# sarpel/wakeword_trainer_home

Measured on AMD Instinct MI355X. Metric: training samples/sec (16kHz x 1.5s clips), higher is better.
Workload: dtype bf16; 1 GPU; BASELINE config 2: cnn_small + log-mel(40) + SpecAugment, fwd/bwd + clip + AdamW, 16 kHz x 1.5 s clips resident in HBM; batch_per_gpu=512, activation_storage=bf16, arithmetic=f32, global_batch=512, n_samples=24000, parallelism=single, ranks_seen=1, hip_graph=False

## Files before the change

### wakeword_trainer_home_amd/csrc/ww_conv_fwd.hip

```cpp
#include "ww_internal.h"
#include "ww_act.h"

namespace {

typedef float floatx16 __attribute__((ext_vector_type(16)));

__device__ __forceinline__ float bnrelu(float y, float s, float t) {
    const float z = fmaf(y, s, t);
    return z < 0.f ? 0.f : z;
}

__device__ __forceinline__ void reduce_stats_slots(float s0, float s1, float q0, float q1, float *sh ,
                                                   float *__restrict__ partial_row) {
    const int tid = threadIdx.x, slot = tid >> 5, cl = tid & 31;
    __syncthreads();
    sh[slot * 128 + 2 * cl] = s0;
    sh[slot * 128 + 2 * cl + 1] = s1;
    sh[slot * 128 + 64 + 2 * cl] = q0;
    sh[slot * 128 + 64 + 2 * cl + 1] = q1;
    __syncthreads();
    if (tid < 128) {
        float t = 0.f;
#pragma unroll
        for (int s = 0; s < 8; ++s) t += sh[s * 128 + tid];
        partial_row[tid] = t;
    }
}

template <typename T>
__global__ __launch_bounds__(256) void k_stem_fwd(const float *__restrict__ x, const float *__restrict__ w, int B,
                                                  int Hin, int Win, int Ho, int Wo, T *__restrict__ y,
                                                  float *__restrict__ partials, int rev) {
    __shared__ float sh[32 * 128];
    extern __shared__ float xs[];
    const int tid = threadIdx.x, px = tid >> 3, c8 = tid & 7;
    const int ld = Win + 2;
    float wr[8][9];
#pragma unroll
    for (int j = 0; j < 8; ++j)
#pragma unroll
        for (int t = 0; t < 9; ++t) wr[j][t] = w[(8 * c8 + j) * 9 + t];
    float s[8], q[8];
#pragma unroll
    for (int j = 0; j < 8; ++j) { s[j] = 0.f; q[j] = 0.f; }
    const long npairs = (long)B * ((Ho + 1) / 2);
    float pre[4];
    auto fetch = [&](long item) {
        if (rev) item = npairs - 1 - item;
        const int fb_ = (int)(item / ((Ho + 1) / 2)), foh = 2 * (int)(item - (long)fb_ * ((Ho + 1) / 2));
        const float *xb = x + (size_t)fb_ * Hin * Win;
#pragma unroll
        for (int k = 0; k < 4; ++k) {
            const int i = tid + 256 * k;
            const int r = i / ld, c = i - r * ld;
            const int ih = 2 * foh - 1 + r, iw = c - 1;
            pre[k] = (i < 5 * ld && ih >= 0 && ih < Hin && iw >= 0 && iw < Win) ? xb[(size_t)ih * Win + iw] : 0.f;
        }
    };
    const bool ahead = 5 * ld <= 4 * 256;
    if (ahead && (long)blockIdx.x < npairs) fetch(blockIdx.x);
    for (long pr = blockIdx.x; pr < npairs; pr += gridDim.x) {
        const long prm = rev ? npairs - 1 - pr : pr;
        const int b = (int)(prm / ((Ho + 1) / 2)), oh0 = 2 * (int)(prm - (long)b * ((Ho + 1) / 2));
        __syncthreads();
        if (ahead) {
#pragma unroll
            for (int k = 0; k < 4; ++k)
                if (tid + 256 * k < 5 * ld) xs[tid + 256 * k] = pre[k];
        } else {
            const float *xb = x + (size_t)b * Hin * Win;
            for (int i = tid; i < 5 * ld; i += 256) {
                const int r = i / ld, c = i - r * ld;
                const int ih = 2 * oh0 - 1 + r, iw = c - 1;
                xs[i] = (ih >= 0 && ih < Hin && iw >= 0 && iw < Win) ? xb[(size_t)ih * Win + iw] : 0.f;
            }
        }
        __syncthreads();
        if (ahead && pr + gridDim.x < npairs) fetch(pr + gridDim.x);
        const int nrow = min(2, Ho - oh0);
        for (int it = px; it < nrow * Wo; it += 32) {
            const int rr = it >= Wo ? 1 : 0, ow = it - rr * Wo;
            float acc[8];
#pragma unroll
            for (int j = 0; j < 8; ++j) acc[j] = 0.f;
#pragma unroll
            for (int kh = 0; kh < 3; ++kh)
#pragma unroll
                for (int kw = 0; kw < 3; ++kw) {
                    const float v = xs[(2 * rr + kh) * ld + 2 * ow + kw];
#pragma unroll
                    for (int j = 0; j < 8; ++j) acc[j] = fmaf(v, wr[j][kh * 3 + kw], acc[j]);
                }
            T *dst = y + (((size_t)b * Ho + oh0 + rr) * Wo + ow) * 64 + 8 * c8;
            float4 o0 = Act<T>::round4(make_float4(acc[0], acc[1], acc[2], acc[3]));
            float4 o1 = Act<T>::round4(make_float4(acc[4], acc[5], acc[6], acc[7]));
            Act<T>::st8(dst, o0, o1);
            s[0] += o0.x; s[1] += o0.y; s[2] += o0.z; s[3] += o0.w; s[4] += o1.x; s[5] += o1.y; s[6] += o1.z; s[7] += o1.w;
            q[0] = fmaf(o0.x, o0.x, q[0]); q[1] = fmaf(o0.y, o0.y, q[1]); q[2] = fmaf(o0.z, o0.z, q[2]); q[3] = fmaf(o0.w, o0.w, q[3]);
            q[4] = fmaf(o1.x, o1.x, q[4]); q[5] = fmaf(o1.y, o1.y, q[5]); q[6] = fmaf(o1.z, o1.z, q[6]); q[7] = fmaf(o1.w, o1.w, q[7]);
        }
    }
    if (partials) {
        __syncthreads();
#pragma unroll
        for (int j = 0; j < 8; ++j) {
            sh[px * 128 + 8 * c8 + j] = s[j];
            sh[px * 128 + 64 + 8 * c8 + j] = q[j];
        }
        __syncthreads();
        if (tid < 128) {
            float t = 0.f;
#pragma unroll 8
            for (int i = 0; i < 32; ++i) t += sh[i * 128 + tid];
            partials[(size_t)blockIdx.x * 128 + tid] = t;
        }
    }
}

struct DwGeom {
    int B, H, W, ncs, nseg, hs_len;
    long items;
};

constexpr int DW_HS = 20;

template <typename T>
__device__ __forceinline__ void dw_issue_row(const T *__restrict__ img, int h, int w0, int H, int W, int cl,
                                             typename Act<T>::raw2 (&raw)[6]) {
    const int hh = min(max(h, 0), H - 1);
#pragma unroll
    for (int i = 0; i < 6; ++i) {
        const int wc = min(max(w0 - 1 + i, 0), W - 1);
        raw[i] = Act<T>::ldraw2(img + (uint32_t)((hh * W + wc) * 64 + 2 * cl));
    }
}
template <typename T>
__device__ __forceinline__ void dw_finish_row(const typename Act<T>::raw2 (&raw)[6], int h, int w0, int H, int W,
                                              float2 sc, float2 sf, float2 (&r)[6]) {
    const bool hv = (h >= 0) && (h < H);
#pragma unroll
    for (int i = 0; i < 6; ++i) {
        const int wc = w0 - 1 + i;
        const bool ok = hv && wc >= 0 && wc < W;
        const float2 v = Act<T>::cvt2(raw[i]);
        r[i].x = ok ? bnrelu(v.x, sc.x, sf.x) : 0.f;
        r[i].y = ok ? bnrelu(v.y, sc.y, sf.y) : 0.f;
    }
}

template <typename T>
__device__ __forceinline__ void dw_out_row(T *__restrict__ oimg, int h, int w0, int W, int cl,
                                           const float2 (&top)[6], const float2 (&mid)[6], const float2 (&bot)[6],
                                           const float (&wa)[9], const float (&wb)[9], float &s0, float &s1, float &q0,
                                           float &q1) {
#pragma unroll
    for (int i = 0; i < 4; ++i) {
        float a0 = 0.f, a1 = 0.f;
#pragma unroll
        for (int kw = 0; kw < 3; ++kw) {
            a0 = fmaf(top[i + kw].x, wa[kw], a0);
            a1 = fmaf(top[i + kw].y, wb[kw], a1);
            a0 = fmaf(mid[i + kw].x, wa[3 + kw], a0);
            a1 = fmaf(mid[i + kw].y, wb[3 + kw], a1);
            a0 = fmaf(bot[i + kw].x, wa[6 + kw], a0);
            a1 = fmaf(bot[i + kw].y, wb[6 + kw], a1);
        }
        if (w0 + i < W) {
            const float2 o = Act<T>::round2(make_float2(a0, a1));
            Act<T>::st2(oimg + (uint32_t)((h * W + w0 + i) * 64 + 2 * cl), o);
            s0 += o.x; s1 += o.y;
            q0 = fmaf(o.x, o.x, q0); q1 = fmaf(o.y, o.y, q1);
        }
    }
}

template <typename T>
__global__ __launch_bounds__(256) void k_dw_fwd(const T *__restrict__ yin, const float *__restrict__ ss,
                                                const float *__restrict__ w, DwGeom g, T *__restrict__ y,
                                                float *__restrict__ partials) {
    __shared__ float sh[8 * 128];
    typedef typename Act<T>::raw2 raw2;
    const int tid = threadIdx.x, slot = tid >> 5, cl = tid & 31;
    float wa[9], wb[9];
#pragma unroll
    for (int t = 0; t < 9; ++t) {
        wa[t] = w[(2 * cl) * 9 + t];
        wb[t] = w[(2 * cl + 1) * 9 + t];
    }
    const float2 sc = *reinterpret_cast<const float2 *>(ss + 2 * cl);
    const float2 sf = *reinterpret_cast<const float2 *>(ss + 64 + 2 * cl);
    float s0 = 0.f, s1 = 0.f, q0 = 0.f, q1 = 0.f;
    const size_t img_stride = (size_t)g.H * g.W * 64;
    for (long item = (long)blockIdx.x * 8 + slot; item < g.items; item += (long)gridDim.x * 8) {
        const int cs = (int)(item % g.ncs);
        const long t = item / g.ncs;
        const int seg = (int)(t % g.nseg), b = (int)(t / g.nseg);
        const int w0 = cs * 4, hs = seg * g.hs_len;
        const int he = min(g.H, hs + g.hs_len);
        const T *img = yin + (size_t)b * img_stride;
        T *oimg = y + (size_t)b * img_stride;
        float2 rows[3][6];
        raw2 raw[6], ahead[6];
        dw_issue_row<T>(img, hs - 1, w0, g.H, g.W, cl, raw);
        dw_finish_row<T>(raw, hs - 1, w0, g.H, g.W, sc, sf, rows[0]);
        dw_issue_row<T>(img, hs, w0, g.H, g.W, cl, raw);
        dw_finish_row<T>(raw, hs, w0, g.H, g.W, sc, sf, rows[1]);
        dw_issue_row<T>(img, hs + 1, w0, g.H, g.W, cl, ahead);
#pragma unroll 1
        for (int i0 = 0; i0 < DW_HS; i0 += 3) {
#pragma unroll
          for (int ii = 0; ii < 3; ++ii) {
            const int i = i0 + ii;
            const int h = hs + i;
            if (h < he) {
#pragma unroll
                for (int c = 0; c < 6; ++c) raw[c] = ahead[c];
                if (h + 1 < he) dw_issue_row<T>(img, h + 2, w0, g.H, g.W, cl, ahead);
                dw_finish_row<T>(raw, h + 1, w0, g.H, g.W, sc, sf, rows[(ii + 2) % 3]);
                dw_out_row<T>(oimg, h, w0, g.W, cl, rows[ii % 3], rows[(ii + 1) % 3], rows[(ii + 2) % 3], wa, wb, s0, s1,
                              q0, q1);
            }
          }
        }
    }
    if (partials) reduce_stats_slots(s0, s1, q0, q1, sh, partials + (size_t)blockIdx.x * 128);
}

constexpr int PW_TILE = 128;
constexpr int PW_LD = 68;

template <typename T>
__global__ __launch_bounds__(256) void k_pw_fwd(const T *__restrict__ yin, const float *__restrict__ ss,
                                                const float *__restrict__ w, long M, T *__restrict__ y,
                                                float *__restrict__ partials) {
    extern __shared__ __align__(16) float pw_lds[];
    float *tile = pw_lds;
    float *otile = pw_lds + PW_TILE * PW_LD;
    typedef typename Act<T>::raw4 raw4;
    const int tid = threadIdx.x, lane = tid & 63, wv = tid >> 6;
    const int r = lane & 31, h = lane >> 5;
    const int rh = wv >> 1, n = wv & 1;
    float wreg[32];
#pragma unroll
    for (int s4 = 0; s4 < 8; ++s4) {
        const float4 v = *reinterpret_cast<const float4 *>(w + (size_t)(32 * n + r) * 64 + 32 * h + 4 * s4);
        wreg[4 * s4] = v.x; wreg[4 * s4 + 1] = v.y; wreg[4 * s4 + 2] = v.z; wreg[4 * s4 + 3] = v.w;
    }
    const int c4 = tid & 15;
    const float4 sc = *reinterpret_cast<const float4 *>(ss + 4 * c4);
    const float4 sf = *reinterpret_cast<const float4 *>(ss + 64 + 4 * c4);
    float s1 = 0.f, s2 = 0.f;
    const long ntiles = (M + PW_TILE - 1) / PW_TILE;
    raw4 raw[8];
    auto issue = [&](long ti) {
#pragma unroll
        for (int i = 0; i < 8; ++i) {
            long p = ti * PW_TILE + (tid >> 4) + 16 * i;
            p = p < M ? p : M - 1;
            raw[i] = Act<T>::ldraw4(yin + (size_t)p * 64 + 4 * c4);
        }
    };
    if ((long)blockIdx.x < ntiles) issue(blockIdx.x);
    for (long ti = blockIdx.x; ti < ntiles; ti += gridDim.x) {
        const long p0 = ti * PW_TILE;
#pragma unroll
        for (int i = 0; i < 8; ++i) {
            const int row = (tid >> 4) + 16 * i;
            const bool ok = p0 + row < M;
            const float4 v = Act<T>::cvt4(raw[i]);
            float4 a;
            a.x = ok ? bnrelu(v.x, sc.x, sf.x) : 0.f; a.y = ok ? bnrelu(v.y, sc.y, sf.y) : 0.f;
            a.z = ok ? bnrelu(v.z, sc.z, sf.z) : 0.f; a.w = ok ? bnrelu(v.w, sc.w, sf.w) : 0.f;
            *reinterpret_cast<float4 *>(tile + row * PW_LD + 4 * c4) = a;
        }
        __syncthreads();
        if (ti + gridDim.x < ntiles) issue(ti + gridDim.x);
#pragma unroll
        for (int t = 0; t < 2; ++t) {
            const int rbase = 64 * rh + 32 * t;
            float a[32];
#pragma unroll
            for (int j = 0; j < 8; ++j) {
                const float4 v = *reinterpret_cast<const float4 *>(tile + (rbase + r) * PW_LD + 32 * h + 4 * j);
                a[4 * j] = v.x; a[4 * j + 1] = v.y; a[4 * j + 2] = v.z; a[4 * j + 3] = v.w;
            }
            floatx16 acc = {0.f};
#pragma unroll
            for (int s = 0; s < 32; ++s) acc = __builtin_amdgcn_mfma_f32_32x32x2f32(a[s], wreg[s], acc, 0, 0, 0);
#pragma unroll
            for (int reg = 0; reg < 16; ++reg) {
                const int prow = rbase + (reg & 3) + 8 * (reg >> 2) + 4 * h;
                const float v = Act<T>::round1(acc[reg]);
                if constexpr (Act<T>::is_f32) {
                    if (p0 + prow < M) y[(size_t)(p0 + prow) * 64 + 32 * n + r] = v;
                } else {
                    otile[prow * PW_LD + 32 * n + r] = v;
                }
                s1 += v;
                s2 = fmaf(v, v, s2);
            }
        }
        __syncthreads();
        if constexpr (!Act<T>::is_f32) {
#pragma unroll
            for (int i = 0; i < 8; ++i) {
                const int row = (tid >> 4) + 16 * i;
                if (p0 + row < M)
                    Act<T>::st4(y + (size_t)(p0 + row) * 64 + 4 * c4,
                                *reinterpret_cast<const float4 *>(otile + row * PW_LD + 4 * c4));
            }
        }
    }
    if (partials) {
        s1 += __shfl_xor(s1, 32);
        s2 += __shfl_xor(s2, 32);
        __syncthreads();
        float *sh = tile;
        if (h == 0) {
            sh[wv * 64 + r] = s1;
            sh[wv * 64 + 32 + r] = s2;
        }
        __syncthreads();
        if (tid < 128) {
            const int kind = tid >> 6, c = tid & 63, nn = c >> 5, rr = c & 31;
            partials[(size_t)blockIdx.x * 128 + tid] = sh[nn * 64 + kind * 32 + rr] + sh[(2 + nn) * 64 + kind * 32 + rr];
        }
    }
}

constexpr int PWH_LD = 72;

template <typename H>
__global__ __launch_bounds__(256) void k_pw_fwd_bf16(const H *__restrict__ yin, const float *__restrict__ ss,
                                                     const float *__restrict__ w, long M, H *__restrict__ y,
                                                     float *__restrict__ partials, int rev) {
    extern __shared__ __align__(16) unsigned char pwh_lds[];
    H *atile = reinterpret_cast<H *>(pwh_lds);
    H *otile = atile + PW_TILE * PWH_LD;
    typedef Act<H> A16;
    typedef typename H16<H>::x8 bf16x8;
    const int tid = threadIdx.x, lane = tid & 63, wv = tid >> 6;
    const int r = lane & 31, h = lane >> 5;
    const int rh = wv >> 1, n = wv & 1;
    bf16x8 wb[4];
#pragma unroll
    for (int t = 0; t < 4; ++t) {
        float v[8];
#pragma unroll
        for (int j = 0; j < 8; ++j) v[j] = w[(size_t)(32 * n + r) * 64 + 16 * t + 8 * h + j];
        wb[t] = ww_pack8<H>(v);
    }
    const int c4 = tid & 15;
    const float4 sc = *reinterpret_cast<const float4 *>(ss + 4 * c4);
    const float4 sf = *reinterpret_cast<const float4 *>(ss + 64 + 4 * c4);
    float s1 = 0.f, s2 = 0.f;
    const long ntiles = (M + PW_TILE - 1) / PW_TILE;
    typename A16::raw4 raw[8];
    auto issue = [&](long ti) {
        if (rev) ti = ntiles - 1 - ti;
#pragma unroll
        for (int i = 0; i < 8; ++i) {
            long p = ti * PW_TILE + (tid >> 4) + 16 * i;
            p = p < M ? p : M - 1;
            raw[i] = A16::ldraw4_nt(yin + (size_t)p * 64 + 4 * c4);
        }
    };
    if ((long)blockIdx.x < ntiles) issue(blockIdx.x);
    for (long ti = blockIdx.x; ti < ntiles; ti += gridDim.x) {
        const long p0 = (rev ? ntiles - 1 - ti : ti) * PW_TILE;
#pragma unroll
        for (int i = 0; i < 8; ++i) {
            const int row = (tid >> 4) + 16 * i;
            const bool ok = p0 + row < M;
            const float4 v = A16::cvt4(raw[i]);
            const float a0 = ok ? bnrelu(v.x, sc.x, sf.x) : 0.f, a1 = ok ? bnrelu(v.y, sc.y, sf.y) : 0.f;
            const float a2 = ok ? bnrelu(v.z, sc.z, sf.z) : 0.f, a3 = ok ? bnrelu(v.w, sc.w, sf.w) : 0.f;
            *reinterpret_cast<uint2 *>(atile + row * PWH_LD + 4 * c4) = make_uint2(A16::pack2(a0, a1), A16::pack2(a2, a3));
        }
        __syncthreads();
        if (ti + gridDim.x < ntiles) issue(ti + gridDim.x);
#pragma unroll
        for (int t2 = 0; t2 < 2; ++t2) {
            const int rbase = 64 * rh + 32 * t2;
            floatx16 acc = {0.f};
#pragma unroll
            for (int t = 0; t < 4; ++t) {
                const bf16x8 a = *reinterpret_cast<const bf16x8 *>(atile + (rbase + r) * PWH_LD + 16 * t + 8 * h);
                acc = H16<H>::mfma32(a, wb[t], acc);
            }
#pragma unroll
            for (int reg = 0; reg < 16; ++reg) {
                const int prow = rbase + (reg & 3) + 8 * (reg >> 2) + 4 * h;
                const float v = A16::round1(acc[reg]);
                otile[prow * PWH_LD + 32 * n + r] = (H)v;
                s1 += v;
                s2 = fmaf(v, v, s2);
            }
        }
        __syncthreads();
#pragma unroll
        for (int i = 0; i < 8; ++i) {
            const int row = (tid >> 4) + 16 * i;
            if (p0 + row < M)
                *reinterpret_cast<uint2 *>(y + (size_t)(p0 + row) * 64 + 4 * c4) =
                    *reinterpret_cast<const uint2 *>(otile + row * PWH_LD + 4 * c4);
        }
    }
    if (partials) {
        s1 += __shfl_xor(s1, 32);
        s2 += __shfl_xor(s2, 32);
        __syncthreads();
        float *sh = reinterpret_cast<float *>(otile);
        if (h == 0) {
            sh[wv * 64 + r] = s1;
            sh[wv * 64 + 32 + r] = s2;
        }
        __syncthreads();
        if (tid < 128) {
            const int kind = tid >> 6, c = tid & 63, nn = c >> 5, rr = c & 31;
            partials[(size_t)blockIdx.x * 128 + tid] = sh[nn * 64 + kind * 32 + rr] + sh[(2 + nn) * 64 + kind * 32 + rr];
        }
    }
}

template <typename T>
__global__ __launch_bounds__(1024) void k_gap_fwd(const T *__restrict__ y, const float *__restrict__ ss,
                                                  const float *__restrict__ mr, int HW, float *__restrict__ pool) {
    __shared__ __align__(16) float sh[64 * 192];
    const int tid = threadIdx.x, slot = tid >> 4, cl = tid & 15, b = blockIdx.x;
    const float4 sc = *reinterpret_cast<const float4 *>(ss + 4 * cl);
    const float4 sf = *reinterpret_cast<const float4 *>(ss + 64 + 4 * cl);
    const float4 mu = *reinterpret_cast<const float4 *>(mr + 4 * cl);
    const float4 rs = *reinterpret_cast<const float4 *>(mr + 64 + 4 * cl);
    const T *yb = y + (size_t)b * HW * 64 + 4 * cl;
    float4 a = make_float4(0.f, 0.f, 0.f, 0.f), h = a, c = a;
    auto one = [](float v, float scv, float sfv, float muv, float rsv, float &av, float &hv, float &cv) {
        const float z = fmaf(v, scv, sfv);
        av += z < 0.f ? 0.f : z;
        if (z > 0.f) { hv += (v - muv) * rsv; cv += 1.f; }
    };
    for (int p0 = slot; p0 < HW; p0 += 8 * 64) {
        typename Act<T>::raw4 r[8];
#pragma unroll
        for (int u = 0; u < 8; ++u) r[u] = Act<T>::ldraw4_nt(yb + (size_t)min(p0 + 64 * u, HW - 1) * 64);
#pragma unroll
        for (int u = 0; u < 8; ++u)
            if (p0 + 64 * u < HW) {
                const float4 v = Act<T>::cvt4(r[u]);
                one(v.x, sc.x, sf.x, mu.x, rs.x, a.x, h.x, c.x);
                one(v.y, sc.y, sf.y, mu.y, rs.y, a.y, h.y, c.y);
                one(v.z, sc.z, sf.z, mu.z, rs.z, a.z, h.z, c.z);
                one(v.w, sc.w, sf.w, mu.w, rs.w, a.w, h.w, c.w);
            }
    }
    *reinterpret_cast<float4 *>(sh + slot * 192 + 4 * cl) = a;
    *reinterpret_cast<float4 *>(sh + slot * 192 + 64 + 4 * cl) = h;
    *reinterpret_cast<float4 *>(sh + slot * 192 + 128 + 4 * cl) = c;
    __syncthreads();
    if (tid < 192) {
        float t = 0.f;
#pragma unroll 8
        for (int s = 0; s < 64; ++s) t += sh[s * 192 + tid];
        pool[(size_t)b * 192 + tid] = t;
    }
}

__global__ __launch_bounds__(256) void k_head_fwd(const float *__restrict__ pool, int B, int HW,
                                                  const float *__restrict__ fc_w, const float *__restrict__ fc_b,
                                                  float drop_scale, uint64_t drop_thresh, int use_dropout,
                                                  uint32_t seed_lo, uint32_t seed_hi, uint32_t step_lo, uint32_t step_hi,
                                                  uint64_t sample_offset, float *__restrict__ pd,
                                                  float *__restrict__ logits, const ww_step_ctl *__restrict__ ctl) {
    const int lane = threadIdx.x & 63, b = blockIdx.x * 4 + (threadIdx.x >> 6);
    if (b >= B) return;
    ww_step_resolve(ctl, step_lo, step_hi, step_lo, step_hi);
    float v = pool[(size_t)b * 192 + lane] / (float)HW;
    if (use_dropout) {
        uint32_t rr[4];
        ww_philox(step_lo, step_hi, (uint32_t)(sample_offset + (uint64_t)b), (WW_TAG_DROPOUT << 24) | (uint32_t)(lane >> 2),
                  seed_lo, seed_hi, rr);
        const uint32_t d = rr[lane & 3];
        v = ((uint64_t)d >= drop_thresh) ? v * drop_scale : 0.f;
    }
    pd[(size_t)b * 64 + lane] = v;
    float l0 = v * fc_w[lane], l1 = v * fc_w[64 + lane];
#pragma unroll
    for (int o = 32; o > 0; o >>= 1) {
        l0 += __shfl_xor(l0, o);
        l1 += __shfl_xor(l1, o);
    }
    if (lane == 0) {
        logits[(size_t)b * 2] = l0 + fc_b[0];
        logits[(size_t)b * 2 + 1] = l1 + fc_b[1];
    }
}

int finish_bn(ww_ctx *ctx, const float *partials, int rows, double count, const ww_bn_t *bn, float *ss_out,
              float *mr_out, hipStream_t st) {
    ww_prof_scope ps_(ctx, WW_K_FINALIZE, st);
    if (bn->training) return ww_launch_bn_fwd_finalize(partials, rows, count, bn, ss_out, mr_out, st);
    return ww_launch_bn_eval_ss(bn, ss_out, mr_out, st);
}

int check_bn(const char *who, const ww_bn_t *bn, const float *ss_out, const float *mr_out, const void *scratch) {
    WW_REQUIRE(bn && bn->gamma && bn->beta && ss_out && mr_out, WW_E_INVALID, "%s: null BatchNorm argument", who);
    WW_REQUIRE(bn->training ? scratch != nullptr : (bn->running_mean && bn->running_var), WW_E_INVALID,
               "%s: training needs scratch, eval needs running statistics", who);
    return WW_OK;
}

int check_act(const char *who, int act_dtype) {
    WW_REQUIRE(act_dtype == WW_ACT_F32 || act_dtype == WW_ACT_BF16 || act_dtype == WW_ACT_F16, WW_E_INVALID, "%s: unknown act_dtype %d", who,
               act_dtype);
    return WW_OK;
}

template <typename T>
int launch_stem_fwd(ww_ctx *ctx, const float *x, const float *w, int B, int Hin, int Win, void *y, float *partials,
                    int *grid_out, hipStream_t st) {
    const int Ho = (Hin + 1) / 2, Wo = (Win + 1) / 2;
    const long nrows = (long)B * ((Ho + 1) / 2);
    const size_t smem = (size_t)5 * (Win + 2) * sizeof(float);
    const int grid = ww_occupancy_grid((const void *)k_stem_fwd<T>, 256, smem, nrows, WW_MAX_PARTIALS);
    {
        ww_prof_scope ps_(ctx, WW_K_STEM_FWD, st);
        static const int rev = ww_env_int("WW_STEM_FWD_REV", 1);
        hipLaunchKernelGGL(k_stem_fwd<T>, dim3(grid), dim3(256), smem, st, x, w, B, Hin, Win, Ho, Wo, (T *)y, partials, rev);
    }
    WW_LAUNCH_CHECK();
    *grid_out = grid;
    return WW_OK;
}

template <typename T>
int launch_dw_fwd(ww_ctx *ctx, const void *y_in, const float *ss_in, const float *w, const DwGeom &g, void *y,
                  float *partials, int *grid_out, hipStream_t st) {
    const long nblk = (g.items + 7) / 8;
    const int grid = ww_occupancy_grid((const void *)k_dw_fwd<T>, 256, 0, nblk, WW_MAX_PARTIALS);
    {
        ww_prof_scope ps_(ctx, WW_K_DW_FWD, st);
        hipLaunchKernelGGL(k_dw_fwd<T>, dim3(grid), dim3(256), 0, st, (const T *)y_in, ss_in, w, g, (T *)y, partials);
    }
    WW_LAUNCH_CHECK();
    *grid_out = grid;
    return WW_OK;
}

template <typename H>
int launch_pw_fwd_bf16(ww_ctx *ctx, const void *y_in, const float *ss_in, const float *w, long M, void *y,
                       float *partials, int *grid_out, hipStream_t st) {
    const long ntiles = (M + PW_TILE - 1) / PW_TILE;
    const size_t smem = (size_t)2 * PW_TILE * PWH_LD * 2;
    const int grid = ww_occupancy_grid((const void *)k_pw_fwd_bf16<H>, 256, smem, ntiles, WW_MAX_PARTIALS);
    {
        ww_prof_scope ps_(ctx, WW_K_PW_FWD, st);
        static const int rev = ww_env_int("WW_PW_FWD_REV", 1);
        hipLaunchKernelGGL(k_pw_fwd_bf16<H>, dim3(grid), dim3(256), smem, st, (const H *)y_in, ss_in, w, M, (H *)y, partials, rev);
    }
    WW_LAUNCH_CHECK();
    *grid_out = grid;
    return WW_OK;
}

template <typename T>
int launch_pw_fwd(ww_ctx *ctx, const void *y_in, const float *ss_in, const float *w, long M, void *y, float *partials,
                  int *grid_out, hipStream_t st) {
    const long ntiles = (M + PW_TILE - 1) / PW_TILE;
    const size_t smem = (size_t)(Act<T>::is_f32 ? 1 : 2) * PW_TILE * PW_LD * sizeof(float);
    WW_HIP(hipFuncSetAttribute((const void *)k_pw_fwd<T>, hipFuncAttributeMaxDynamicSharedMemorySize, (int)smem));
    const int grid = ww_occupancy_grid((const void *)k_pw_fwd<T>, 256, smem, ntiles, WW_MAX_PARTIALS);
    {
        ww_prof_scope ps_(ctx, WW_K_PW_FWD, st);
        hipLaunchKernelGGL(k_pw_fwd<T>, dim3(grid), dim3(256), smem, st, (const T *)y_in, ss_in, w, M, (T *)y, partials);
    }
    WW_LAUNCH_CHECK();
    *grid_out = grid;
    return WW_OK;
}

}

extern "C" int ww_conv_stem_fwd(ww_ctx *ctx, int act_dtype, const float *x, const float *w, int B, int Hin, int Win,
                                void *y, const ww_bn_t *bn, float *ss_out, float *mr_out, void *scratch,
                                ww_stream_t stream) {
    WW_REQUIRE(ctx && x && w && y, WW_E_INVALID, "ww_conv_stem_fwd: null argument");
    WW_REQUIRE(B >= 1 && Hin >= 1 && Win >= 1, WW_E_INVALID, "ww_conv_stem_fwd: bad shape (%d,%d,%d)", B, Hin, Win);
    int rc = check_bn("ww_conv_stem_fwd", bn, ss_out, mr_out, scratch);
    if (rc || (rc = check_act("ww_conv_stem_fwd", act_dtype))) return rc;
    hipStream_t st = (hipStream_t)stream;
    float *partials = bn->training ? (float *)scratch : nullptr;
    int grid = 0;
    rc = act_dtype == WW_ACT_BF16  ? launch_stem_fwd<ww_bf16>(ctx, x, w, B, Hin, Win, y, partials, &grid, st)
         : act_dtype == WW_ACT_F16 ? launch_stem_fwd<ww_f16>(ctx, x, w, B, Hin, Win, y, partials, &grid, st)
                                   : launch_stem_fwd<float>(ctx, x, w, B, Hin, Win, y, partials, &grid, st);
    if (rc) return rc;
    return finish_bn(ctx, partials, grid, (double)B * ((Hin + 1) / 2) * ((Win + 1) / 2), bn, ss_out, mr_out, st);
}

extern "C" int ww_dwconv3x3_fwd(ww_ctx *ctx, int act_dtype, const void *y_in, const float *ss_in, const float *w,
                                int B, int H, int W, void *y, const ww_bn_t *bn, float *ss_out, float *mr_out,
                                void *scratch, ww_stream_t stream) {
    WW_REQUIRE(ctx && y_in && ss_in && w && y, WW_E_INVALID, "ww_dwconv3x3_fwd: null argument");
    WW_REQUIRE(B >= 1 && H >= 1 && W >= 1, WW_E_INVALID, "ww_dwconv3x3_fwd: bad shape (%d,%d,%d)", B, H, W);
    WW_REQUIRE((long)H * W * 64 < (1L << 31), WW_E_UNSUPPORTED, "ww_dwconv3x3_fwd: one image of %d x %d x 64 exceeds 2^31 elements", H, W);
    int rc = check_bn("ww_dwconv3x3_fwd", bn, ss_out, mr_out, scratch);
    if (rc || (rc = check_act("ww_dwconv3x3_fwd", act_dtype))) return rc;
    DwGeom g;
    g.B = B; g.H = H; g.W = W;
    g.ncs = (W + 3) / 4;
    g.nseg = (H + DW_HS - 1) / DW_HS;
    g.hs_len = (H + g.nseg - 1) / g.nseg;
    g.items = (long)B * g.nseg * g.ncs;
    hipStream_t st = (hipStream_t)stream;
    float *partials = bn->training ? (float *)scratch : nullptr;
    int grid = 0;
    rc = act_dtype == WW_ACT_BF16  ? launch_dw_fwd<ww_bf16>(ctx, y_in, ss_in, w, g, y, partials, &grid, st)
         : act_dtype == WW_ACT_F16 ? launch_dw_fwd<ww_f16>(ctx, y_in, ss_in, w, g, y, partials, &grid, st)
                                   : launch_dw_fwd<float>(ctx, y_in, ss_in, w, g, y, partials, &grid, st);
    if (rc) return rc;
    return finish_bn(ctx, partials, grid, (double)B * H * W, bn, ss_out, mr_out, st);
}

extern "C" int ww_pwconv1x1_fwd(ww_ctx *ctx, int act_dtype, const void *y_in, const float *ss_in, const float *w,
                                int B, int H, int W, void *y, const ww_bn_t *bn, float *ss_out, float *mr_out,
                                void *scratch, ww_stream_t stream) {
    WW_REQUIRE(ctx && y_in && ss_in && w && y, WW_E_INVALID, "ww_pwconv1x1_fwd: null argument");
    WW_REQUIRE(B >= 1 && H >= 1 && W >= 1, WW_E_INVALID, "ww_pwconv1x1_fwd: bad shape (%d,%d,%d)", B, H, W);
    int rc = check_bn("ww_pwconv1x1_fwd", bn, ss_out, mr_out, scratch);
    if (rc || (rc = check_act("ww_pwconv1x1_fwd", act_dtype))) return rc;
    const long M = (long)B * H * W;
    hipStream_t st = (hipStream_t)stream;
    float *partials = bn->training ? (float *)scratch : nullptr;
    int grid = 0;
    rc = act_dtype == WW_ACT_BF16  ? launch_pw_fwd_bf16<ww_bf16>(ctx, y_in, ss_in, w, M, y, partials, &grid, st)
         : act_dtype == WW_ACT_F16 ? launch_pw_fwd_bf16<ww_f16>(ctx, y_in, ss_in, w, M, y, partials, &grid, st)
                                   : launch_pw_fwd<float>(ctx, y_in, ss_in, w, M, y, partials, &grid, st);
    if (rc) return rc;
    return finish_bn(ctx, partials, grid, (double)M, bn, ss_out, mr_out, st);
}

extern "C" int ww_gap_fwd(ww_ctx *ctx, int act_dtype, const void *y, const float *ss, const float *mr, int B, int H,
                          int W, float *pool, ww_stream_t stream) {
    WW_REQUIRE(ctx && y && ss && mr && pool, WW_E_INVALID, "ww_gap_fwd: null argument");
    WW_REQUIRE(B >= 1 && H >= 1 && W >= 1, WW_E_INVALID, "ww_gap_fwd: bad shape (%d,%d,%d)", B, H, W);
    int rc = check_act("ww_gap_fwd", act_dtype);
    if (rc) return rc;
    hipStream_t st = (hipStream_t)stream;
    {
        ww_prof_scope ps_(ctx, WW_K_GAP_FWD, st);
        if (act_dtype == WW_ACT_BF16)
            hipLaunchKernelGGL(k_gap_fwd<ww_bf16>, dim3(B), dim3(1024), 0, st, (const ww_bf16 *)y, ss, mr, H * W, pool);
        else if (act_dtype == WW_ACT_F16)
            hipLaunchKernelGGL(k_gap_fwd<ww_f16>, dim3(B), dim3(1024), 0, st, (const ww_f16 *)y, ss, mr, H * W, pool);
        else
            hipLaunchKernelGGL(k_gap_fwd<float>, dim3(B), dim3(1024), 0, st, (const float *)y, ss, mr, H * W, pool);
    }
    WW_LAUNCH_CHECK();
    return WW_OK;
}

extern "C" int ww_head_fwd(ww_ctx *ctx, const float *pool, int B, int HW, const float *fc_w, const float *fc_b,
                           float dropout_p, int training, uint64_t seed, uint64_t step, uint64_t sample_offset,
                           float *pd, float *logits, ww_stream_t stream) {
    WW_REQUIRE(ctx && pool && fc_w && fc_b && pd && logits, WW_E_INVALID, "ww_head_fwd: null argument");
    WW_REQUIRE(B >= 1 && HW >= 1, WW_E_INVALID, "ww_head_fwd: bad shape (%d,%d)", B, HW);
    WW_REQUIRE(dropout_p >= 0.f && dropout_p < 1.f, WW_E_INVALID, "ww_head_fwd: dropout_p=%f not in [0,1)", dropout_p);
    const int use_dropout = training && dropout_p > 0.f;
    const float scale = (float)(1.0 / (1.0 - (double)dropout_p));
    ww_prof_scope ps_(ctx, WW_K_HEAD_LOSS, (hipStream_t)stream);
    hipLaunchKernelGGL(k_head_fwd, dim3((B + 3) / 4), dim3(256), 0, (hipStream_t)stream, pool, B, HW, fc_w, fc_b,
                       scale, ww_prob_threshold((double)dropout_p), use_dropout, (uint32_t)seed, (uint32_t)(seed >> 32),
                       (uint32_t)step, (uint32_t)(step >> 32), sample_offset, pd, logits, ctx->step_ctl);
    WW_LAUNCH_CHECK();
    return WW_OK;
}
```

### wakeword_trainer_home_amd/csrc/ww_ctx.hip

```cpp
#include <math.h>
#include <stdarg.h>
#include <stdlib.h>
#include <string.h>
#include <vector>

#include "ww_internal.h"
#include <algorithm>

static thread_local char g_err[512] = "";

void ww_set_error(const char *fmt, ...) {
    va_list ap;
    va_start(ap, fmt);
    vsnprintf(g_err, sizeof(g_err), fmt, ap);
    va_end(ap);
}

extern "C" const char *ww_last_error(void) { return g_err; }
extern "C" int ww_abi_version(void) { return WW_ABI_VERSION; }

extern "C" uint64_t ww_prob_threshold(double p) {
    double t = floor(p * 4294967296.0);
    if (!(t > 0.0)) return 0;
    if (t > 4294967296.0) t = 4294967296.0;
    return (uint64_t)t;
}

extern "C" void ww_philox4x32_10(const uint32_t ctr[4], const uint32_t key[2], uint32_t out[4]) {
    ww_philox(ctr[0], ctr[1], ctr[2], ctr[3], key[0], key[1], out);
}

extern "C" int ww_feat_num_frames(int n_samples, int hop) {
    if (hop <= 0 || n_samples < 0) return WW_E_INVALID;
    return 1 + n_samples / hop;
}

extern "C" int ww_ctx_create(int device, ww_ctx **out) {
    WW_REQUIRE(out != nullptr, WW_E_INVALID, "ww_ctx_create: out is null");
    int ndev = 0;
    WW_HIP(hipGetDeviceCount(&ndev));
    WW_REQUIRE(device >= 0 && device < ndev, WW_E_INVALID, "ww_ctx_create: device %d not in [0,%d)", device, ndev);
    hipDeviceProp_t prop;
    WW_HIP(hipGetDeviceProperties(&prop, device));
    WW_REQUIRE(strncmp(prop.gcnArchName, "gfx950", 6) == 0, WW_E_UNSUPPORTED,
               "ww_ctx_create: libwwhip is built for gfx950 only, device %d is %s", device, prop.gcnArchName);
    ww_ctx *c = new ww_ctx();
    c->device = device;
    c->tables = nullptr;
    c->prof_mask = 0;
    c->step_ctl = nullptr;
    c->logmel_wgs = 0;
    c->tw16k = nullptr;
    c->norm_partials = nullptr;
    c->defer_on = 0;
    c->deferred = new std::vector<ww_reduce_item>();
    c->prof_recs = new std::vector<ww_prof_rec>();
    c->prof_free = new std::vector<ww_prof_rec>();
    *out = c;
    return WW_OK;
}

__global__ void k_step_ctl_advance(ww_step_ctl *ctl) {
    ctl->step += 1;
    ctl->parity ^= 1;
}

extern "C" int ww_ctx_bind_step_ctl(ww_ctx *ctx, const ww_step_ctl *ctl_dev) {
    WW_REQUIRE(ctx != nullptr, WW_E_INVALID, "ww_ctx_bind_step_ctl: ctx is null");
    WW_REQUIRE(((uintptr_t)ctl_dev & 7) == 0, WW_E_INVALID, "ww_ctx_bind_step_ctl: the control block must be 8-byte aligned");
    ctx->step_ctl = ctl_dev;
    return WW_OK;
}

extern "C" int ww_ctx_set_logmel_workgroups(ww_ctx *ctx, int n) {
    WW_REQUIRE(ctx != nullptr, WW_E_INVALID, "ww_ctx_set_logmel_workgroups: ctx is null");
    WW_REQUIRE(n >= 0, WW_E_INVALID, "ww_ctx_set_logmel_workgroups: n=%d must be >= 0", n);
    ctx->logmel_wgs = n;
    return WW_OK;
}

extern "C" int ww_step_ctl_advance(ww_ctx *ctx, ww_stream_t stream) {
    WW_REQUIRE(ctx && ctx->step_ctl, WW_E_INVALID, "ww_step_ctl_advance: no control block is bound");
    hipLaunchKernelGGL(k_step_ctl_advance, dim3(1), dim3(1), 0, (hipStream_t)stream, const_cast<ww_step_ctl *>(ctx->step_ctl));
    WW_LAUNCH_CHECK();
    return WW_OK;
}

static void free_tables(ww_feat_tables *t) {
    while (t) {
        ww_feat_tables *n = t->next;
        (void)hipFree(t->window);
        (void)hipFree(t->twiddle);
        (void)hipFree(t->mel_start);
        (void)hipFree(t->mel_len);
        (void)hipFree(t->mel_off);
        (void)hipFree(t->mel_w);
        if (t->melq_tab) (void)hipFree(t->melq_tab);
        if (t->melq_w) (void)hipFree(t->melq_w);
        if (t->dct) (void)hipFree(t->dct);
        if (t->dct_t) (void)hipFree(t->dct_t);
        delete t;
        t = n;
    }
}

extern "C" int ww_ctx_destroy(ww_ctx *ctx) {
    if (!ctx) return WW_OK;
    free_tables(ctx->tables);
    if (ctx->tw16k) (void)hipFree(ctx->tw16k);
    if (ctx->norm_partials) (void)hipFree(ctx->norm_partials);
    for (auto *v : {ctx->prof_recs, ctx->prof_free}) {
        for (auto &r : *v) { (void)hipEventDestroy(r.a); (void)hipEventDestroy(r.b); }
        delete v;
    }
    delete ctx->deferred;
    delete ctx;
    return WW_OK;
}

constexpr int RED_MAX = 64;
struct ReduceBatch { ww_reduce_item it[RED_MAX]; int first_block[RED_MAX + 1]; int count; };
constexpr int RED_COLS = 256;
__global__ __launch_bounds__(256) void k_reduce_items(ReduceBatch b) {
    __shared__ double sh[3][64][4];
    int i = 0;
    while (i + 1 < b.count && (int)blockIdx.x >= b.first_block[i + 1]) ++i;
    const float *__restrict__ part = b.it[i].part;
    float *__restrict__ dst = b.it[i].dst;
    const long n = b.it[i].n;
    const int splits = b.it[i].splits, acc = b.it[i].accumulate;
    const int c4 = threadIdx.x & 63, q = threadIdx.x >> 6;
    const long i0 = ((long)((int)blockIdx.x - b.first_block[i]) * 64 + c4) * 4;
    const bool vec = (n & 3) == 0 && (((uintptr_t)part | (uintptr_t)dst) & 15) == 0;
    double s0 = 0.0, s1 = 0.0, s2 = 0.0, s3 = 0.0;
    if (i0 < n) {
        if (vec) {
            for (int z0 = q; z0 < splits; z0 += 32) {
                float4 v[8];
#pragma unroll
                for (int u = 0; u < 8; ++u) v[u] = *reinterpret_cast<const float4 *>(part + (long)min(z0 + 4 * u, splits - 1) * n + i0);
#pragma unroll
                for (int u = 0; u < 8; ++u)
                    if (z0 + 4 * u < splits) { s0 += v[u].x; s1 += v[u].y; s2 += v[u].z; s3 += v[u].w; }
            }
        } else {
            for (int z = q; z < splits; z += 4) {
                const float *p = part + (long)z * n + i0;
                s0 += p[0];
                if (i0 + 1 < n) s1 += p[1];
                if (i0 + 2 < n) s2 += p[2];
                if (i0 + 3 < n) s3 += p[3];
            }
        }
    }
    if (q > 0) { sh[q - 1][c4][0] = s0; sh[q - 1][c4][1] = s1; sh[q - 1][c4][2] = s2; sh[q - 1][c4][3] = s3; }
    __syncthreads();
    if (q != 0 || i0 >= n) return;
#pragma unroll
    for (int k = 0; k < 3; ++k) { s0 += sh[k][c4][0]; s1 += sh[k][c4][1]; s2 += sh[k][c4][2]; s3 += sh[k][c4][3]; }
    if (vec) {
        float4 o = make_float4((float)s0, (float)s1, (float)s2, (float)s3);
        if (acc) { const float4 c = *reinterpret_cast<const float4 *>(dst + i0); o.x += c.x; o.y += c.y; o.z += c.z; o.w += c.w; }
        *reinterpret_cast<float4 *>(dst + i0) = o;
    } else {
        const double sv[4] = {s0, s1, s2, s3};
        for (int k = 0; k < 4 && i0 + k < n; ++k) dst[i0 + k] = acc ? dst[i0 + k] + (float)sv[k] : (float)sv[k];
    }
}
extern "C" int ww_ctx_set_deferred_reduce(ww_ctx *ctx, int on) {
    WW_REQUIRE(ctx != nullptr, WW_E_INVALID, "ww_ctx_set_deferred_reduce: ctx is null");
    ctx->defer_on = on != 0;
    return WW_OK;
}
extern "C" int ww_deferred_reduce_pending(ww_ctx *ctx) { return ctx ? (int)ctx->deferred->size() : 0; }
extern "C" int ww_deferred_reduce_discard(ww_ctx *ctx) {
    WW_REQUIRE(ctx != nullptr, WW_E_INVALID, "ww_deferred_reduce_discard: ctx is null");
    ctx->deferred->clear();
    ctx->defer_on = 0;
    return WW_OK;
}
extern "C" int ww_deferred_reduce_flush(ww_ctx *ctx, ww_stream_t stream) {
    WW_REQUIRE(ctx != nullptr, WW_E_INVALID, "ww_deferred_reduce_flush: ctx is null");
    std::vector<ww_reduce_item> &q = *ctx->deferred;
    for (size_t base = 0; base < q.size(); base += RED_MAX) {
        ReduceBatch b;
        b.count = (int)std::min<size_t>(RED_MAX, q.size() - base);
        int blocks = 0;
        for (int i = 0; i < b.count; ++i) {
            b.it[i] = q[base + i];
            b.first_block[i] = blocks;
            blocks += (int)((b.it[i].n + RED_COLS - 1) / RED_COLS);
        }
        for (int i = b.count; i <= RED_MAX; ++i) b.first_block[i] = blocks;
        for (int i = b.count; i < RED_MAX; ++i) b.it[i] = ww_reduce_item{nullptr, nullptr, 0, 0, 0};
        if (blocks > 0) hipLaunchKernelGGL(k_reduce_items, dim3(blocks), dim3(256), 0, (hipStream_t)stream, b);
    }
    q.clear();
    WW_LAUNCH_CHECK();
    return WW_OK;
}

static double hz_to_mel(double f) { return 2595.0 * log10(1.0 + f / 700.0); }
static double mel_to_hz(double m) { return 700.0 * (pow(10.0, m / 2595.0) - 1.0); }

template <typename T>
static int upload(T **dptr, const std::vector<T> &h) {
    size_t bytes = (h.empty() ? 1 : h.size()) * sizeof(T);
    WW_HIP(hipMalloc((void **)dptr, bytes));
    if (!h.empty()) WW_HIP(hipMemcpy(*dptr, h.data(), h.size() * sizeof(T), hipMemcpyHostToDevice));
    return WW_OK;
}

struct MelTables {
    std::vector<int32_t> start, len, off, qtab;
    std::vector<float> w, qw;
    int max_len = 0;
};
static void build_mel_tables(const ww_feat_cfg *cfg, MelTables &mt) {
    const int n_fft = cfg->n_fft, n_bins = n_fft / 2 + 1, M = cfg->n_mels;
    const double sr = cfg->sample_rate;
    const double f_min = cfg->f_min, f_max = cfg->f_max > 0.f ? cfg->f_max : sr / 2.0;
    std::vector<int32_t> &qtab = mt.qtab;
    std::vector<float> &w = mt.w, &qw = mt.qw;
    int &max_len = mt.max_len;
    std::vector<double> f_pts(M + 2);
    const double m_lo = hz_to_mel(f_min), m_hi = hz_to_mel(f_max);
    for (int i = 0; i < M + 2; ++i) {
        double m = (i == M + 1) ? m_hi : m_lo + i * ((m_hi - m_lo) / (M + 1));
        f_pts[i] = mel_to_hz(m);
    }
    std::vector<int32_t> &start = mt.start, &len = mt.len, &off = mt.off;
    start.assign(M, 0); len.assign(M, 0); off.assign(M, 0);
    w.clear();
    max_len = 0;
    for (int m = 0; m < M; ++m) {
        int s = -1, e = -1;
        std::vector<float> band;
        for (int k = 0; k < n_bins; ++k) {
            double f = (k == n_bins - 1) ? sr / 2.0 : k * ((sr / 2.0) / (n_bins - 1));
            double down = -(f_pts[m] - f) / (f_pts[m + 1] - f_pts[m]);
            double up = (f_pts[m + 2] - f) / (f_pts[m + 2] - f_pts[m + 1]);
            double v = fmax(0.0, fmin(down, up));
            if (v > 0.0) {
                if (s < 0) s = k;
                e = k;
            }
        }
        if (s < 0) { s = 0; e = -1; }
        start[m] = s;
        len[m] = e - s + 1;
        off[m] = (int32_t)w.size();
        for (int k = s; k <= e; ++k) {
            double f = (k == n_bins - 1) ? sr / 2.0 : k * ((sr / 2.0) / (n_bins - 1));
            double down = -(f_pts[m] - f) / (f_pts[m + 1] - f_pts[m]);
            double up = (f_pts[m + 2] - f) / (f_pts[m + 2] - f_pts[m + 1]);
            w.push_back((float)fmax(0.0, fmin(down, up)));
        }
        if (len[m] > max_len) max_len = len[m];
    }
    qtab.assign(WW_MELQ_TAB, 0);
    qw.clear();
    if (n_fft <= WW_NFFT) {
        const int r = WW_NFFT / n_fft;
        struct Unit { int quad, g0, g1; };
        const int NQ = (M + 3) / 4, Pmin = (NQ + 15) / 16;
        std::vector<Unit> quads;
        for (int q = 0; q < NQ; ++q) {
            int s = WW_NFFT / 2 + 1, e = 0;
            for (int m = 4 * q; m < std::min(M, 4 * q + 4); ++m)
                if (len[m] > 0) { s = std::min(s, r * start[m]); e = std::max(e, r * (start[m] + len[m] - 1) + 1); }
            if (e <= s) { s = 0; e = 0; }
            quads.push_back(Unit{q, s / 8, (e + 7) / 8});
        }
        std::vector<Unit> units;
        std::vector<int> order;
        int best = -1;
        for (int P = Pmin; P <= WW_MELQ_MAX_PASSES; ++P) {
            std::vector<int> pieces(NQ, 1);
            auto longest = [&](int q) { return pieces[q] >= 8 ? 0 : (quads[q].g1 - quads[q].g0 + pieces[q] - 1) / pieces[q]; };
            int fill = 0;
            for (int n = NQ; n < 16 * P; ++n) {
                int big = 0;
                for (int q = 1; q < NQ; ++q)
                    if (longest(q) > longest(big)) big = q;
                if (pieces[big] >= 8) ++fill; else ++pieces[big];
            }
            std::vector<Unit> us;
            for (int q = 0; q < NQ; ++q) {
                const int g = quads[q].g1 - quads[q].g0;
                for (int i = 0; i < pieces[q]; ++i) us.push_back(Unit{q, quads[q].g0 + g * i / pieces[q], quads[q].g0 + g * (i + 1) / pieces[q]});
                if (q == NQ - 1)
                    for (int i = 0; i < fill; ++i) us.push_back(Unit{q, quads[q].g1, quads[q].g1});
            }
            std::vector<int> ord(us.size());
            for (size_t i = 0; i < ord.size(); ++i) ord[i] = (int)i;
            std::stable_sort(ord.begin(), ord.end(), [&](int x, int y) { return us[x].g1 - us[x].g0 > us[y].g1 - us[y].g0; });
            int total = 0;
            for (int p = 0; p < P; ++p) total += 8 * (us[ord[16 * p]].g1 - us[ord[16 * p]].g0);
            if (best < 0 || total < best) { best = total; units = us; order = ord; }
        }
        const int P = (int)units.size() / 16;
        qtab[0] = P; qtab[1] = NQ;
        for (int p = 0; p < P; ++p) {
            const int steps = 8 * (units[order[16 * p]].g1 - units[order[16 * p]].g0);
            qtab[2 + 2 * p] = steps;
            qtab[3 + 2 * p] = (int32_t)qw.size();
            for (int b = 0; b < 16; ++b) {
                qtab[10 + 32 * p + 2 * b] = 8 * units[order[16 * p + b]].g0;
                qtab[11 + 32 * p + 2 * b] = order[16 * p + b];
            }
            for (int t = 0; t < steps; ++t)
                for (int lane = 0; lane < 64; ++lane) {
                    const Unit &u = units[order[16 * p + (lane >> 2)]];
                    const int m = 4 * u.quad + (lane & 3), j = 8 * u.g0 + t;
                    const int k = j / r;
                    const bool in = m < M && j < 8 * u.g1 && j % r == 0 && k >= start[m] && k < start[m] + len[m];
                    qw.push_back(in ? 0.25f * w[off[m] + (k - start[m])] : 0.f);
                }
        }
        for (int q = 0, i = 0; q <= NQ; ++q) {
            while (i < (int)units.size() && units[i].quad < q) ++i;
            qtab[138 + q] = i;
        }
    }
}

extern "C" int ww_feat_mel_tables(const ww_feat_cfg *cfg, int32_t *start, int32_t *len, float *w, int w_cap, int32_t *n_w,
                                  int32_t *melq_tab, float *melq_w, int melq_cap, int32_t *n_melq_w) {
    WW_REQUIRE(cfg && start && len && n_w, WW_E_INVALID, "ww_feat_mel_tables: null argument");
    WW_REQUIRE(cfg->n_fft >= 64 && cfg->n_fft <= 4096 && (cfg->n_fft & (cfg->n_fft - 1)) == 0 && cfg->n_mels >= 1 &&
               cfg->n_mels <= WW_MAX_MELS && cfg->sample_rate > 0, WW_E_INVALID, "ww_feat_mel_tables: bad configuration");
    MelTables mt;
    build_mel_tables(cfg, mt);
    memcpy(start, mt.start.data(), mt.start.size() * sizeof(int32_t));
    memcpy(len, mt.len.data(), mt.len.size() * sizeof(int32_t));
    *n_w = (int32_t)mt.w.size();
    if (w) {
        WW_REQUIRE(w_cap >= (int)mt.w.size(), WW_E_INVALID, "ww_feat_mel_tables: w holds %d floats, %d needed", w_cap, (int)mt.w.size());
        memcpy(w, mt.w.data(), mt.w.size() * sizeof(float));
    }
    if (n_melq_w) *n_melq_w = (int32_t)mt.qw.size();
    if (melq_tab) memcpy(melq_tab, mt.qtab.data(), WW_MELQ_TAB * sizeof(int32_t));
    if (melq_w) {
        WW_REQUIRE(melq_cap >= (int)mt.qw.size(), WW_E_INVALID, "ww_feat_mel_tables: melq_w holds %d floats, %d needed", melq_cap, (int)mt.qw.size());
        memcpy(melq_w, mt.qw.data(), mt.qw.size() * sizeof(float));
    }
    return WW_OK;
}

int ww_get_feat_tables(ww_ctx *ctx, const ww_feat_cfg *cfg, ww_feat_tables **out) {
    for (ww_feat_tables *t = ctx->tables; t; t = t->next) {
        if (memcmp(&t->cfg, cfg, sizeof(ww_feat_cfg)) == 0) {
            *out = t;
            return WW_OK;
        }
    }
    const int n_fft = cfg->n_fft, M = cfg->n_mels;
    const int n_tab = n_fft < WW_NFFT ? WW_NFFT : n_fft, lead = (n_tab - n_fft) / 2;
    std::vector<float> win(n_tab, 0.f);
    std::vector<float2> tw(n_tab);
    for (int i = 0; i < n_fft; ++i) win[lead + i] = (float)(0.5 - 0.5 * cos(2.0 * M_PI * i / n_fft));
    for (int i = 0; i < n_tab; ++i)
        tw[i] = make_float2((float)cos(2.0 * M_PI * i / n_tab), (float)(-sin(2.0 * M_PI * i / n_tab)));
    MelTables mt;
    build_mel_tables(cfg, mt);
    const std::vector<int32_t> &start = mt.start, &len = mt.len, &off = mt.off, &qtab = mt.qtab;
    const std::vector<float> &w = mt.w, &qw = mt.qw;
    const int max_len = mt.max_len;
    std::vector<float> dct;
    if (cfg->n_mfcc > 0) {
        dct.resize((size_t)cfg->n_mfcc * M);
        for (int c = 0; c < cfg->n_mfcc; ++c)
            for (int m = 0; m < M; ++m) {
                double v = cos(M_PI / M * (m + 0.5) * c) * sqrt(2.0 / M);
                if (c == 0) v *= 1.0 / sqrt(2.0);
                dct[(size_t)c * M + m] = (float)v;
            }
    }
    ww_feat_tables *t = new ww_feat_tables();
    memset(t, 0, sizeof(*t));
    t->cfg = *cfg;
    t->n_melq_w = (int32_t)qw.size();
    t->max_len = max_len;
    t->n_mel_w = (int32_t)w.size();
    int rc;
    if ((rc = upload(&t->window, win)) || (rc = upload(&t->twiddle, tw)) || (rc = upload(&t->mel_start, start)) ||
        (rc = upload(&t->mel_len, len)) || (rc = upload(&t->mel_off, off)) || (rc = upload(&t->mel_w, w)) ||
        (rc = upload(&t->melq_tab, qtab)) || (rc = upload(&t->melq_w, qw))) {
        free_tables(t);
        return rc;
    }
    std::vector<float> dct_t(dct.size());
    for (int c = 0; c < cfg->n_mfcc; ++c)
        for (int m = 0; m < M; ++m) dct_t[(size_t)m * cfg->n_mfcc + c] = dct[(size_t)c * M + m];
    if (cfg->n_mfcc > 0 && ((rc = upload(&t->dct, dct)) || (rc = upload(&t->dct_t, dct_t)))) {
        free_tables(t);
        return rc;
    }
    t->next = ctx->tables;
    ctx->tables = t;
    *out = t;
    return WW_OK;
}

extern "C" size_t ww_layer_scratch_bytes(void) {
    return (size_t)(WW_STAT_SLAB_FLOATS + WW_DW_SLAB_FLOATS) * sizeof(float);
}


__device__ __forceinline__ void ww_colgroup_sum(const float *__restrict__ partials, int rows, int cg, double (*sh)[16],
                                                double *tot ) {
    const int q = threadIdx.x & 3, part = threadIdx.x >> 2;
    {
        const int col = (q < 2 ? 8 * cg + 4 * q : 64 + 8 * cg + 4 * (q - 2));
        double a0 = 0.0, a1 = 0.0, a2 = 0.0, a3 = 0.0;
        for (int r0 = part; r0 < rows; r0 += 4 * 256) {
            float4 v[4];
#pragma unroll
            for (int u = 0; u < 4; ++u) v[u] = *reinterpret_cast<const float4 *>(partials + (size_t)min(r0 + 256 * u, rows - 1) * 128 + col);
#pragma unroll
            for (int u = 0; u < 4; ++u)
                if (r0 + 256 * u < rows) { a0 += (double)v[u].x; a1 += (double)v[u].y; a2 += (double)v[u].z; a3 += (double)v[u].w; }
        }
        sh[part][4 * q] = a0; sh[part][4 * q + 1] = a1; sh[part][4 * q + 2] = a2; sh[part][4 * q + 3] = a3;
    }
    __syncthreads();
    const int c = threadIdx.x & 15, seg = (threadIdx.x >> 4) & 15;
    double t2 = 0.0;
    if (threadIdx.x < 256) {
#pragma unroll
        for (int p = 0; p < 16; ++p) t2 += sh[16 * seg + p][c];
    }
    __syncthreads();
    if (threadIdx.x < 256) sh[seg][c] = t2;
    __syncthreads();
    if (threadIdx.x < 16) {
        double t = 0.0;
#pragma unroll
        for (int p = 0; p < 16; ++p) t += sh[p][threadIdx.x];
        tot[threadIdx.x] = t;
    }
    __syncthreads();
}

__global__ __launch_bounds__(1024) void k_bn_fwd_finalize(const float *__restrict__ partials, int rows,
                                                          double count, ww_bn_t bn, float *__restrict__ ss,
                                                          float *__restrict__ mr) {
    __shared__ double sh[256][16];
    __shared__ double tot[16];
    float g_c = 0.f, b_c = 0.f, rm_c = 0.f, rv_c = 1.f;
    if (threadIdx.x < 8) {
        const int c = 8 * blockIdx.x + threadIdx.x;
        g_c = bn.gamma[c]; b_c = bn.beta[c];
        if (bn.running_mean) { rm_c = bn.running_mean[c]; rv_c = bn.running_var[c]; }
    }
    ww_colgroup_sum(partials, rows, blockIdx.x, sh, tot);
    if (threadIdx.x < 8) {
        const int c = 8 * blockIdx.x + threadIdx.x;
        const double mean = tot[threadIdx.x] / count;
        double var = tot[8 + threadIdx.x] / count - mean * mean;
        if (var < 0.0) var = 0.0;
        const double rstd = 1.0 / sqrt(var + (double)bn.eps);
        const double scale = (double)g_c * rstd;
        ss[c] = (float)scale;
        ss[64 + c] = (float)((double)b_c - mean * scale);
        mr[c] = (float)mean;
        mr[64 + c] = (float)rstd;
        if (bn.running_mean) {
            const double m = bn.momentum;
            const double unb = count > 1.0 ? var * count / (count - 1.0) : var;
            bn.running_mean[c] = (float)((1.0 - m) * (double)rm_c + m * mean);
            bn.running_var[c] = (float)((1.0 - m) * (double)rv_c + m * unb);
        }
    }
}

__global__ void k_bn_eval_ss(ww_bn_t bn, float *__restrict__ ss, float *__restrict__ mr) {
    const int c = threadIdx.x;
    if (c < 64) {
        const double rstd = 1.0 / sqrt((double)bn.running_var[c] + (double)bn.eps);
        const double scale = (double)bn.gamma[c] * rstd;
        ss[c] = (float)scale;
        ss[64 + c] = (float)((double)bn.beta[c] - (double)bn.running_mean[c] * scale);
        mr[c] = bn.running_mean[c];
        mr[64 + c] = (float)rstd;
    }
}

__device__ __forceinline__ void bn_bwd_finalize_group(const float *__restrict__ partials, int rows, double count, int cg,
                                                      const float *__restrict__ gamma, const float *__restrict__ mr,
                                                      float *__restrict__ coef, float *__restrict__ dgamma,
                                                      float *__restrict__ dbeta, double (*sh)[16], double *tot) {
    float mean_c = 0.f, rstd_c = 0.f, g_c = 0.f;
    if (threadIdx.x < 8) { const int c = 8 * cg + threadIdx.x; mean_c = mr[c]; rstd_c = mr[64 + c]; g_c = gamma[c]; }
    ww_colgroup_sum(partials, rows, cg, sh, tot);
    if (threadIdx.x < 8) {
        const int c = 8 * cg + threadIdx.x;
        const double s1 = tot[threadIdx.x], s2 = tot[8 + threadIdx.x];
        const double mean = mean_c, rstd = rstd_c, g = g_c;
        const double c1 = s1 / count, c2 = s2 / count;
        const double A = g * rstd;
        coef[c] = (float)A;
        coef[64 + c] = (float)(-A * rstd * c2);
        coef[128 + c] = (float)(A * (mean * rstd * c2 - c1));
        dgamma[c] = (float)s2;
        dbeta[c] = (float)s1;
    }
}

__global__ __launch_bounds__(1024) void k_bn_bwd_finalize(const float *__restrict__ partials, int rows,
                                                          double count, const float *__restrict__ gamma,
                                                          const float *__restrict__ mr, float *__restrict__ coef,
                                                          float *__restrict__ dgamma, float *__restrict__ dbeta) {
    __shared__ double sh[256][16];
    __shared__ double tot[16];
    bn_bwd_finalize_group(partials, rows, count, blockIdx.x, gamma, mr, coef, dgamma, dbeta, sh, tot);
}

__device__ __forceinline__ void colsum_body(const float *__restrict__ partials, int rows, int cols,
                                            float *__restrict__ out, int blk, double *sh ) {
    const int c4 = threadIdx.x & 15, part = threadIdx.x >> 4;
    const int col = blk * 64 + 4 * c4;
    double a0 = 0.0, a1 = 0.0, a2 = 0.0, a3 = 0.0;
    if (col < cols)
        for (int r0 = part; r0 < rows; r0 += 8 * 64) {
            float4 v[8];
#pragma unroll
            for (int u = 0; u < 8; ++u) v[u] = *reinterpret_cast<const float4 *>(partials + (size_t)min(r0 + 64 * u, rows - 1) * cols + col);
#pragma unroll
            for (int u = 0; u < 8; ++u)
                if (r0 + 64 * u < rows) { a0 += (double)v[u].x; a1 += (double)v[u].y; a2 += (double)v[u].z; a3 += (double)v[u].w; }
        }
    sh[part * 64 + 4 * c4] = a0; sh[part * 64 + 4 * c4 + 1] = a1;
    sh[part * 64 + 4 * c4 + 2] = a2; sh[part * 64 + 4 * c4 + 3] = a3;
    __syncthreads();
    if (threadIdx.x < 64 && blk * 64 + threadIdx.x < cols) {
        double t = 0.0;
#pragma unroll 8
        for (int p = 0; p < 64; ++p) t += sh[p * 64 + threadIdx.x];
        out[blk * 64 + threadIdx.x] = (float)t;
    }
}

__global__ __launch_bounds__(1024) void k_colsum(const float *__restrict__ partials, int rows, int cols,
                                                 float *__restrict__ out) {
    __shared__ double sh[64 * 64];
    colsum_body(partials, rows, cols, out, blockIdx.x, sh);
}

__global__ __launch_bounds__(1024) void k_bwd_finalize(const float *__restrict__ stat, int rows, double count,
                                                       const float *__restrict__ gamma, const float *__restrict__ mr,
                                                       float *__restrict__ coef, float *__restrict__ dgamma,
                                                       float *__restrict__ dbeta, const float *__restrict__ dwp,
                                                       int cols, float *__restrict__ dw) {
    __shared__ double sh[64 * 64];
    __shared__ double tot[16];
    if (blockIdx.x < 8) {
        bn_bwd_finalize_group(stat, rows, count, blockIdx.x, gamma, mr, coef, dgamma, dbeta,
                              reinterpret_cast<double(*)[16]>(sh), tot);
    } else {
        colsum_body(dwp, rows, cols, dw, blockIdx.x - 8, sh);
    }
}

int ww_launch_bn_fwd_finalize(const float *partials, int rows, double count, const ww_bn_t *bn, float *ss_out,
                              float *mr_out, hipStream_t st) {
    hipLaunchKernelGGL(k_bn_fwd_finalize, dim3(8), dim3(1024), 0, st, partials, rows, count, *bn, ss_out, mr_out);
    WW_LAUNCH_CHECK();
    return WW_OK;
}
int ww_launch_bn_eval_ss(const ww_bn_t *bn, float *ss_out, float *mr_out, hipStream_t st) {
    hipLaunchKernelGGL(k_bn_eval_ss, dim3(1), dim3(64), 0, st, *bn, ss_out, mr_out);
    WW_LAUNCH_CHECK();
    return WW_OK;
}
int ww_launch_bn_bwd_finalize(const float *partials, int rows, double count, const float *gamma,
                              const float *mr, float *coef_out, float *dgamma, float *dbeta, hipStream_t st) {
    hipLaunchKernelGGL(k_bn_bwd_finalize, dim3(8), dim3(1024), 0, st, partials, rows, count, gamma, mr, coef_out,
                       dgamma, dbeta);
    WW_LAUNCH_CHECK();
    return WW_OK;
}
int ww_launch_bwd_finalize(const float *stat, int rows, double count, const float *gamma, const float *mr,
                           float *coef, float *dgamma, float *dbeta, const float *dwp, int cols, float *dw,
                           hipStream_t st) {
    hipLaunchKernelGGL(k_bwd_finalize, dim3(8 + (cols + 63) / 64), dim3(1024), 0, st, stat, rows, count, gamma, mr, coef,
                       dgamma, dbeta, dwp, cols, dw);
    WW_LAUNCH_CHECK();
    return WW_OK;
}
int ww_launch_colsum(const float *partials, int rows, int cols, float *out, hipStream_t st) {
    hipLaunchKernelGGL(k_colsum, dim3((cols + 63) / 64), dim3(1024), 0, st, partials, rows, cols, out);
    WW_LAUNCH_CHECK();
    return WW_OK;
}

__global__ __launch_bounds__(1024) void k_grad_norm_clip(float *__restrict__ g, size_t n, float max_norm,
                                                         float *__restrict__ norm_out,
                                                         ww_step_stats *__restrict__ stats) {
    __shared__ double sh[1024];
    __shared__ float coef_sh;
    double acc = 0.0;
    for (size_t i = threadIdx.x; i < n; i += 1024) {
        const double v = g[i];
        acc += v * v;
    }
    sh[threadIdx.x] = acc;
    __syncthreads();
    for (int s = 512; s > 0; s >>= 1) {
        if ((int)threadIdx.x < s) sh[threadIdx.x] += sh[threadIdx.x + s];
        __syncthreads();
    }
    if (threadIdx.x == 0) {
        const float norm = (float)sqrt(sh[0]);
        if (norm_out) *norm_out = norm;
        if (stats) {
            stats->grad_norm = norm;
            if (!isfinite(norm)) stats->found_inf = 1.0f;
        }
        float c = 1.0f;
        if (max_norm > 0.f) {
            c = max_norm / (norm + 1e-6f);
            if (c > 1.0f) c = 1.0f;
        }
        coef_sh = c;
    }
    __syncthreads();
    const float c = coef_sh;
    if (max_norm > 0.f)
        for (size_t i = threadIdx.x; i < n; i += 1024) g[i] *= c;
}

__global__ __launch_bounds__(1024) void k_sumsq_partials(const float *__restrict__ g, size_t n, double *__restrict__ parts) {
    __shared__ double sh[1024];
    const size_t per = (n + gridDim.x - 1) / gridDim.x;
    const size_t lo = (size_t)blockIdx.x * per, hi = lo + per < n ? lo + per : n;
    double acc = 0.0;
    for (size_t i = lo + threadIdx.x; i < hi; i += 1024) {
        const double v = g[i];
        acc += v * v;
    }
    sh[threadIdx.x] = acc;
    __syncthreads();
    for (int s = 512; s > 0; s >>= 1) {
        if ((int)threadIdx.x < s) sh[threadIdx.x] += sh[threadIdx.x + s];
        __syncthreads();
    }
    if (threadIdx.x == 0) parts[blockIdx.x] = sh[0];
}

__global__ __launch_bounds__(256) void k_norm_clip_apply(float *__restrict__ g, size_t n, const double *__restrict__ parts,
                                                         int nparts, float max_norm, float *__restrict__ norm_out,
                                                         ww_step_stats *__restrict__ stats) {
    double t = 0.0;
    for (int i = 0; i < nparts; ++i) t += parts[i];
    const float norm = (float)sqrt(t);
    if (blockIdx.x == 0 && threadIdx.x == 0) {
        if (norm_out) *norm_out = norm;
        if (stats) {
            stats->grad_norm = norm;
            if (!isfinite(norm)) stats->found_inf = 1.0f;
        }
    }
    if (!(max_norm > 0.f)) return;
    float c = max_norm / (norm + 1e-6f);
    if (c > 1.0f) c = 1.0f;
    for (size_t i = (size_t)blockIdx.x * 256 + threadIdx.x; i < n; i += (size_t)gridDim.x * 256) g[i] *= c;
}

int ww_launch_sumsq_partials(ww_ctx *ctx, const float *g, size_t n, int *parts_out, hipStream_t st) {
    if (!ctx->norm_partials) WW_HIP(hipMalloc((void **)&ctx->norm_partials, WW_NORM_PARTS * sizeof(double)));
    const int parts = (int)std::min<size_t>(WW_NORM_PARTS, (n + 4095) / 4096);
    hipLaunchKernelGGL(k_sumsq_partials, dim3(parts), dim3(1024), 0, st, g, n, ctx->norm_partials);
    WW_LAUNCH_CHECK();
    *parts_out = parts;
    return WW_OK;
}

extern "C" int ww_grad_norm_clip(ww_ctx *ctx, float *flat_grads, size_t n, float max_norm, float *norm_out,
                                 ww_step_stats *stats, ww_stream_t stream) {
    WW_REQUIRE(ctx && flat_grads, WW_E_INVALID, "ww_grad_norm_clip: null argument");
    if (n == 0) return WW_OK;
    hipStream_t st = (hipStream_t)stream;
    ww_prof_scope ps_(ctx, WW_K_CLIP, st);
    if (n <= (size_t)1 << 16) {
        hipLaunchKernelGGL(k_grad_norm_clip, dim3(1), dim3(1024), 0, st, flat_grads, n, max_norm, norm_out, stats);
        WW_LAUNCH_CHECK();
        return WW_OK;
    }
    int parts = 0;
    const int rc = ww_launch_sumsq_partials(ctx, flat_grads, n, &parts, st);
    if (rc) return rc;
    const int grid = (int)std::min<size_t>((n + 255) / 256, 256 * 8);
    hipLaunchKernelGGL(k_norm_clip_apply, dim3(grid), dim3(256), 0, st, flat_grads, n, ctx->norm_partials, parts, max_norm,
                       norm_out, stats);
    WW_LAUNCH_CHECK();
    return WW_OK;
}

int ww_occupancy_grid(const void *fn, int block, size_t smem, long want, int cap) {
    static int n_cu = 0;
    struct Entry { const void *fn; size_t smem; int per_cu; };
    static Entry cache[32];
    static int n_cache = 0;
    if (!n_cu) {
        int dev = 0;
        hipDeviceProp_t prop;
        if (hipGetDevice(&dev) == hipSuccess && hipGetDeviceProperties(&prop, dev) == hipSuccess)
            n_cu = prop.multiProcessorCount;
        else
            n_cu = 256;
    }
    int per_cu = 0;
    for (int i = 0; i < n_cache; ++i)
        if (cache[i].fn == fn && cache[i].smem == smem) per_cu = cache[i].per_cu;
    if (!per_cu) {
        if (hipOccupancyMaxActiveBlocksPerMultiprocessor(&per_cu, fn, block, smem) != hipSuccess || per_cu < 1) per_cu = 1;
        if (n_cache < 32) cache[n_cache++] = Entry{fn, smem, per_cu};
    }
    long gsz = (long)per_cu * n_cu;
    if (gsz > cap) gsz = cap;
    if (gsz > want) gsz = want;
    return (int)(gsz < 1 ? 1 : gsz);
}

static const char *k_class_names[WW_K_NCLASS] = {"logmel_specaug", "conv_stem_fwd", "dwconv3x3_fwd", "pwconv1x1_fwd",
                                                 "gap_fwd", "head_loss", "pwconv1x1_bwd", "dwconv3x3_bwd",
                                                 "conv_stem_bwd", "finalize", "grad_norm_clip", "audio_augment", "linear_mfma", "gru", "nhwc_layers", "lstm"};
extern "C" int ww_prof_num_classes(void) { return WW_K_NCLASS; }
extern "C" const char *ww_prof_class_name(int cls) { return (cls >= 0 && cls < WW_K_NCLASS) ? k_class_names[cls] : ""; }
extern "C" int ww_prof_enable(ww_ctx *ctx, uint32_t class_mask) {
    WW_REQUIRE(ctx != nullptr, WW_E_INVALID, "ww_prof_enable: ctx is null");
    ctx->prof_mask = class_mask;
    return WW_OK;
}
extern "C" int ww_prof_collect(ww_ctx *ctx, float *ms_sum, int32_t *count) {
    WW_REQUIRE(ctx && ms_sum && count, WW_E_INVALID, "ww_prof_collect: null argument");
    for (int i = 0; i < WW_K_NCLASS; ++i) { ms_sum[i] = 0.f; count[i] = 0; }
    for (auto &r : *ctx->prof_recs) {
        WW_HIP(hipEventSynchronize(r.b));
        float ms = 0.f;
        WW_HIP(hipEventElapsedTime(&ms, r.a, r.b));
        ms_sum[r.cls] += ms;
        count[r.cls] += 1;
        ctx->prof_free->push_back(r);
    }
    ctx->prof_recs->clear();
    return WW_OK;
}
```

### wakeword_trainer_home_amd/csrc/ww_internal.h

```cpp
#pragma once
#include <hip/hip_runtime.h>
#include <stdint.h>
#include <stdio.h>
#include <vector>
#include "wwhip.h"

#define WW_NFFT 1024
#define WW_NBINS 513
#define WW_MAX_MELS 128
#define WW_MELQ_MAX_PASSES 4
#define WW_MAX_MASKS 16
#define WW_FRAMES_PER_BLOCK 16
#define WW_MAX_HOP 512
#define WW_NORM_PARTS 256

void ww_set_error(const char *fmt, ...);

#define WW_REQUIRE(cond, code, ...)          \
    do {                                     \
        if (!(cond)) {                       \
            ww_set_error(__VA_ARGS__);       \
            return (code);                   \
        }                                    \
    } while (0)

#define WW_HIP(expr)                                                                      \
    do {                                                                                  \
        hipError_t e_ = (expr);                                                           \
        if (e_ != hipSuccess) {                                                           \
            ww_set_error("%s failed: %s (%s:%d)", #expr, hipGetErrorString(e_), __FILE__, \
                         __LINE__);                                                       \
            return WW_E_HIP;                                                              \
        }                                                                                 \
    } while (0)

#define WW_LAUNCH_CHECK()                                                                   \
    do {                                                                                    \
        hipError_t e_ = hipGetLastError();                                                  \
        if (e_ != hipSuccess) {                                                             \
            ww_set_error("kernel launch failed: %s (%s:%d)", hipGetErrorString(e_), __FILE__, \
                         __LINE__);                                                         \
            return WW_E_HIP;                                                                \
        }                                                                                   \
    } while (0)

struct ww_feat_tables {
    ww_feat_cfg cfg;
    float *window;
    float2 *twiddle;
    int32_t *mel_start;
    int32_t *mel_len;
    int32_t *mel_off;
    float *mel_w;
    float *dct;
    float *dct_t;
    int32_t max_len;
    int32_t n_mel_w;
    int32_t *melq_tab;
    float *melq_w;
    int32_t n_melq_w;
    ww_feat_tables *next;
};

enum {
    WW_K_LOGMEL = 0, WW_K_STEM_FWD, WW_K_DW_FWD, WW_K_PW_FWD, WW_K_GAP_FWD, WW_K_HEAD_LOSS, WW_K_PW_BWD, WW_K_DW_BWD,
    WW_K_STEM_BWD, WW_K_FINALIZE, WW_K_CLIP, WW_K_AUDIO_AUG, WW_K_LINEAR, WW_K_GRU, WW_K_NHWC, WW_K_LSTM,
    WW_K_NCLASS
};
struct ww_prof_rec { int cls; hipEvent_t a, b; };
struct ww_reduce_item { const float *part; float *dst; long n; int splits; int accumulate; };
struct ww_ctx {
    int device;
    ww_feat_tables *tables;
    float2 *tw16k;
    double *norm_partials;
    const ww_step_ctl *step_ctl;
    int logmel_wgs;
    uint32_t prof_mask;
    std::vector<ww_prof_rec> *prof_recs;
    std::vector<ww_prof_rec> *prof_free;
    int defer_on;
    std::vector<ww_reduce_item> *deferred;
};
static inline bool ww_defer(ww_ctx *ctx, const float *part, float *dst, long n, int splits, int accumulate) {
    if (!ctx || !ctx->defer_on) return false;
    ctx->deferred->push_back(ww_reduce_item{part, dst, n, splits, accumulate});
    return true;
}
struct ww_prof_scope {
    ww_ctx *ctx; hipStream_t st; ww_prof_rec r; bool on;
    ww_prof_scope(ww_ctx *c, int cls, hipStream_t s) : ctx(c), st(s), on(false) {
        if (!c || !(c->prof_mask & (1u << cls))) return;
        hipStreamCaptureStatus cs = hipStreamCaptureStatusNone;
        if (hipStreamIsCapturing(s, &cs) != hipSuccess || cs != hipStreamCaptureStatusNone) return;
        if (!c->prof_free->empty()) { r = c->prof_free->back(); c->prof_free->pop_back(); }
        else if (hipEventCreate(&r.a) != hipSuccess || hipEventCreate(&r.b) != hipSuccess) return;
        r.cls = cls;
        on = hipEventRecord(r.a, s) == hipSuccess;
    }
    ~ww_prof_scope() {
        if (!on) return;
        (void)hipEventRecord(r.b, st);
        ctx->prof_recs->push_back(r);
    }
};

int ww_get_feat_tables(ww_ctx *ctx, const ww_feat_cfg *cfg, ww_feat_tables **out);

#define WW_STAT_SLAB_FLOATS (WW_MAX_PARTIALS * 128)
#define WW_DW_SLAB_ROWS 768
#define WW_DW_SLAB_FLOATS (WW_DW_SLAB_ROWS * 4096)

int ww_launch_bn_fwd_finalize(const float *partials, int rows, double count, const ww_bn_t *bn, float *ss_out,
                              float *mr_out, hipStream_t st);
int ww_launch_bn_eval_ss(const ww_bn_t *bn, float *ss_out, float *mr_out, hipStream_t st);
int ww_launch_bn_bwd_finalize(const float *partials, int rows, double count, const float *gamma,
                              const float *mr, float *coef_out, float *dgamma, float *dbeta, hipStream_t st);
int ww_launch_colsum(const float *partials, int rows, int cols, float *out, hipStream_t st);
int ww_launch_bwd_finalize(const float *stat, int rows, double count, const float *gamma, const float *mr,
                           float *coef, float *dgamma, float *dbeta, const float *dwp, int cols, float *dw,
                           hipStream_t st);

int ww_gemm(int mode, const float *A, long a_srow, long a_sk, int a_rows, const float *B, long b_srow, long b_sk, int b_rows,
            int K, float *C, long ldc, const float *bias, int accumulate, int splits, float *part, hipStream_t st,
            ww_ctx *defer_ctx = nullptr, int a16 = 0);
int ww_gemm_seg2(int mode, const float *A, const float *A2, long a_srow, int a_rows, const float *B, const float *B2, long b_sk,
                 int b_rows, int kseg, float *C, long ldc, int accumulate, hipStream_t st, int a16);
int ww_colsum_rows(const float *a, long rows, int cols, float *out, float *part, int chunks, hipStream_t st);
int ww_colsum_pair(const float *a, int rows, int cols, float *out0, float *out1, hipStream_t st);
int ww_colsum_rows_small(const float *a, int rows, int cols, float *out, hipStream_t st);
int ww_occupancy_grid(const void *fn, int block, size_t smem, long want, int cap);
static inline int ww_env_int(const char *name, int dflt) {
    const char *e = getenv(name);
    return e ? atoi(e) : dflt;
}
int ww_stem_bwd_impl(ww_ctx *ctx, int act_dtype, const void *g, const void *y_out, const float *w, const float *coef,
                     const float *x, int B, int Hin, int Win, float *dw, void *scratch, ww_stream_t stream);
int ww_launch_sumsq_partials(ww_ctx *ctx, const float *g, size_t n, int *parts_out, hipStream_t st);

#define WW_TAG_SPECAUG 0u
#define WW_TAG_DROPOUT 1u

__host__ __device__ inline void ww_philox(uint32_t c0, uint32_t c1, uint32_t c2, uint32_t c3, uint32_t k0,
                                          uint32_t k1, uint32_t out[4]) {
#pragma unroll
    for (int r = 0; r < 10; ++r) {
        uint64_t p0 = (uint64_t)0xD2511F53u * c0;
        uint64_t p1 = (uint64_t)0xCD9E8D57u * c2;
        uint32_t hi0 = (uint32_t)(p0 >> 32), lo0 = (uint32_t)p0;
        uint32_t hi1 = (uint32_t)(p1 >> 32), lo1 = (uint32_t)p1;
        uint32_t n0 = hi1 ^ c1 ^ k0, n2 = hi0 ^ c3 ^ k1;
        c0 = n0; c1 = lo1; c2 = n2; c3 = lo0;
        k0 += 0x9E3779B9u;
        k1 += 0xBB67AE85u;
    }
    out[0] = c0; out[1] = c1; out[2] = c2; out[3] = c3;
}

__device__ __forceinline__ void ww_step_resolve(const ww_step_ctl *ctl, uint32_t lo, uint32_t hi, uint32_t &out_lo,
                                                uint32_t &out_hi) {
    uint64_t s = ((uint64_t)hi << 32) | lo;
    if (ctl) s += ctl->step;
    out_lo = (uint32_t)s;
    out_hi = (uint32_t)(s >> 32);
}

struct ww_mask_params {
    int32_t n_f, n_t, f_param, t_param;
    uint64_t f_thresh, t_thresh;
    uint32_t seed_lo, seed_hi, step_lo, step_hi;
    uint64_t sample_offset;
    const ww_step_ctl *ctl;
};

__device__ inline void ww_specaug_mask(const ww_mask_params &mp, uint32_t sample, int k, int F, int T, int &s,
                                       int &w) {
    uint32_t r[4], slo, shi;
    ww_step_resolve(mp.ctl, mp.step_lo, mp.step_hi, slo, shi);
    ww_philox(slo, shi, sample, (WW_TAG_SPECAUG << 24) | (uint32_t)k, mp.seed_lo, mp.seed_hi, r);
    const bool is_f = k < mp.n_f;
    const uint32_t dim = is_f ? (uint32_t)F : (uint32_t)T;
    const uint32_t param = is_f ? (uint32_t)mp.f_param : (uint32_t)mp.t_param;
    const uint32_t pmax = param < dim ? param : dim;
    const uint32_t ww = r[0] % (pmax + 1u);
    const uint32_t ss = r[1] % (dim - ww + 1u);
    const uint64_t thr = is_f ? mp.f_thresh : mp.t_thresh;
    s = (int)ss;
    w = ((uint64_t)r[2] < thr) ? (int)ww : 0;
}
```

### wakeword_trainer_home_amd/csrc/ww_model.hip

```cpp
#include "ww_internal.h"
#include "ww_act.h"
#include <algorithm>

namespace {

constexpr int NL = 9;

struct Layout {
    int Ho, Wo;
    size_t A;
    size_t y[NL], g[2], ss[NL], mr[NL], coef[NL], pool, pd, dpool, scratch, total;
};

Layout make_layout(int B, int F, int T, int act_dtype) {
    Layout L;
    L.Ho = (F + 1) / 2;
    L.Wo = (T + 1) / 2;
    L.A = (size_t)B * L.Ho * L.Wo * 64;
    const size_t esz = act_dtype == WW_ACT_F32 ? 4 : 2;
    size_t o = 0;
    auto takeb = [&](size_t bytes) { size_t r = o; o += (bytes + 255) & ~(size_t)255; return r; };
    auto take = [&](size_t nfloat) { return takeb(nfloat * sizeof(float)); };
    for (int i = 0; i < NL; ++i) L.y[i] = takeb(L.A * esz);
    L.g[0] = takeb(L.A * esz);
    L.g[1] = takeb(L.A * esz);
    for (int i = 0; i < NL; ++i) { L.ss[i] = take(128); L.mr[i] = take(128); L.coef[i] = take(192); }
    L.pool = take((size_t)B * 192);
    L.pd = take((size_t)B * 64);
    L.dpool = take((size_t)B * 64);
    L.scratch = take(WW_STAT_SLAB_FLOATS + WW_DW_SLAB_FLOATS);
    L.total = o;
    return L;
}

inline int widx(int l) { return l == 0 ? 0 : (l & 1 ? 5 + 10 * ((l - 1) / 2) : 10 + 10 * ((l - 2) / 2)); }
inline int bnidx(int l) { return widx(l) + 1; }

ww_bn_t make_bn(void *const *p, int l, int training, float mom, float eps) {
    ww_bn_t bn;
    const int b = bnidx(l);
    bn.gamma = (const float *)p[b];
    bn.beta = (const float *)p[b + 1];
    bn.running_mean = (float *)p[b + 2];
    bn.running_var = (float *)p[b + 3];
    bn.momentum = mom;
    bn.eps = eps;
    bn.training = training;
    return bn;
}

int check_common(const char *who, ww_ctx *ctx, int act_dtype, void *const *params, const void *x, int B, int F, int T,
                 void *ws, size_t ws_bytes, int nparams = WW_CNN_SMALL_NPTR) {
    WW_REQUIRE(act_dtype == WW_ACT_F32 || act_dtype == WW_ACT_BF16 || act_dtype == WW_ACT_F16, WW_E_INVALID, "%s: unknown act_dtype %d", who,
               act_dtype);
    WW_REQUIRE(ctx && params && x && ws, WW_E_INVALID, "%s: null argument", who);
    WW_REQUIRE(B >= 1 && F >= 1 && T >= 1, WW_E_INVALID, "%s: bad shape (%d,1,%d,%d)", who, B, F, T);
    for (int i = 0; i < nparams; ++i)
        WW_REQUIRE(params[i] != nullptr, WW_E_INVALID, "%s: params[%d] is null", who, i);
    const size_t need = ww_cnn_small_workspace_bytes(B, F, T, act_dtype);
    WW_REQUIRE(ws_bytes >= need, WW_E_WORKSPACE, "%s: workspace %zu B < required %zu B", who, ws_bytes, need);
    WW_REQUIRE(((uintptr_t)ws & 255) == 0, WW_E_INVALID, "%s: workspace must be 256-byte aligned", who);
    return WW_OK;
}

int conv_stack_fwd(ww_ctx *ctx, int act_dtype, void *const *params, const float *x, int B, int F, int T, int training,
                   float bn_momentum, float bn_eps, const Layout &L, char *w, ww_stream_t stream) {
    auto Fp = [&](size_t off) { return (float *)(w + off); };
    void *scratch = w + L.scratch;
    ww_bn_t bn = make_bn(params, 0, training, bn_momentum, bn_eps);
    int rc = ww_conv_stem_fwd(ctx, act_dtype, x, (const float *)params[0], B, F, T, w + L.y[0], &bn, Fp(L.ss[0]), Fp(L.mr[0]),
                              scratch, stream);
    if (rc) return rc;
    for (int i = 0; i < 4; ++i) {
        const int ld = 1 + 2 * i, lp = 2 + 2 * i;
        bn = make_bn(params, ld, training, bn_momentum, bn_eps);
        rc = ww_dwconv3x3_fwd(ctx, act_dtype, w + L.y[ld - 1], Fp(L.ss[ld - 1]), (const float *)params[widx(ld)], B, L.Ho,
                              L.Wo, w + L.y[ld], &bn, Fp(L.ss[ld]), Fp(L.mr[ld]), scratch, stream);
        if (rc) return rc;
        bn = make_bn(params, lp, training, bn_momentum, bn_eps);
        rc = ww_pwconv1x1_fwd(ctx, act_dtype, w + L.y[ld], Fp(L.ss[ld]), (const float *)params[widx(lp)], B, L.Ho, L.Wo,
                              w + L.y[lp], &bn, Fp(L.ss[lp]), Fp(L.mr[lp]), scratch, stream);
        if (rc) return rc;
    }
    return WW_OK;
}

int conv_stack_bwd(ww_ctx *ctx, int act_dtype, void *const *params, void *const *grads, const float *x, int B, int F, int T,
                   const Layout &L, char *w, bool from_pool, ww_stream_t stream, int part = WW_BWD_ALL) {
    auto Fp = [&](size_t off) { return (float *)(w + off); };
    auto G = [&](int i) { return (float *)grads[i]; };
    void *scratch = w + L.scratch;
    int rc;
    const int i_hi = part == WW_BWD_EARLY ? 1 : 3, i_lo = part == WW_BWD_LATE ? 2 : 0;
    int cur = (from_pool && i_hi != 3) ? 1 : 0;
    for (int i = i_hi; i >= i_lo; --i) {
        const int ld = 1 + 2 * i, lp = 2 + 2 * i;
        const bool pooled = from_pool && lp == 8;
        const void *gp = pooled ? nullptr : w + L.g[cur];
        const int nxt = pooled ? 0 : cur ^ 1;
        rc = ww_pwconv1x1_bwd(ctx, act_dtype, gp, Fp(L.dpool), w + L.y[lp], Fp(L.ss[lp]), Fp(L.coef[lp]), w + L.y[ld],
                              Fp(L.ss[ld]), Fp(L.mr[ld]), (const float *)params[bnidx(ld)],
                              (const float *)params[widx(lp)], B, L.Ho, L.Wo, w + L.g[nxt], G(widx(lp)), Fp(L.coef[ld]),
                              G(bnidx(ld)), G(bnidx(ld) + 1), scratch, stream);
        if (rc) return rc;
        cur = nxt;
        const int lprev = ld - 1;
        rc = ww_dwconv3x3_bwd(ctx, act_dtype, w + L.g[cur], w + L.y[ld], Fp(L.coef[ld]), w + L.y[lprev], Fp(L.ss[lprev]),
                              Fp(L.mr[lprev]), (const float *)params[bnidx(lprev)], (const float *)params[widx(ld)], B,
                              L.Ho, L.Wo, w + L.g[cur ^ 1], G(widx(ld)), Fp(L.coef[lprev]), G(bnidx(lprev)),
                              G(bnidx(lprev) + 1), scratch, stream);
        if (rc) return rc;
        cur ^= 1;
    }
    if (part == WW_BWD_LATE) return WW_OK;
    return ww_stem_bwd_impl(ctx, act_dtype, w + L.g[cur], w + L.y[0], (const float *)params[0], Fp(L.coef[0]), x, B, F, T, G(0),
                            scratch, stream);
}

template <typename T>
__global__ __launch_bounds__(256) void k_freqpool_fwd(const T *__restrict__ y, const float *__restrict__ ss, int B, int H, int W,
                                                      float *__restrict__ seq) {
    const int grp = threadIdx.x >> 5, cl = threadIdx.x & 31;
    const float2 sc = *reinterpret_cast<const float2 *>(ss + 2 * cl);
    const float2 sf = *reinterpret_cast<const float2 *>(ss + 64 + 2 * cl);
    const float inv = 1.0f / (float)H;
    for (long it = (long)blockIdx.x * 8 + grp; it < (long)B * W; it += (long)gridDim.x * 8) {
        const long b = it / W;
        const int wc = (int)(it % W);
        const T *p = y + ((size_t)b * H * W + wc) * 64 + 2 * cl;
        float a0 = 0.f, a1 = 0.f;
#pragma unroll 4
        for (int h = 0; h < H; ++h) {
            const float2 v = Act<T>::cvt2(Act<T>::ldraw2(p + (size_t)h * W * 64));
            const float z0 = fmaf(v.x, sc.x, sf.x), z1 = fmaf(v.y, sc.y, sf.y);
            a0 += z0 < 0.f ? 0.f : z0;
            a1 += z1 < 0.f ? 0.f : z1;
        }
        *reinterpret_cast<float2 *>(seq + (size_t)it * 64 + 2 * cl) = make_float2(a0 * inv, a1 * inv);
    }
}
template <typename T>
__global__ __launch_bounds__(256) void k_freqpool_bwd(const float *__restrict__ dseq, const T *__restrict__ y,
                                                      const float *__restrict__ ss, const float *__restrict__ mr, int B, int H,
                                                      int W, T *__restrict__ g, float *__restrict__ stat_partials) {
    __shared__ float sh[8 * 128];
    const int grp = threadIdx.x >> 5, cl = threadIdx.x & 31;
    const float2 sc = *reinterpret_cast<const float2 *>(ss + 2 * cl);
    const float2 sf = *reinterpret_cast<const float2 *>(ss + 64 + 2 * cl);
    const float2 mu = *reinterpret_cast<const float2 *>(mr + 2 * cl);
    const float2 rs = *reinterpret_cast<const float2 *>(mr + 64 + 2 * cl);
    const float inv = 1.0f / (float)H;
    float s1a = 0.f, s1b = 0.f, s2a = 0.f, s2b = 0.f;
    for (long it = (long)blockIdx.x * 8 + grp; it < (long)B * W; it += (long)gridDim.x * 8) {
        const long b = it / W;
        const int wc = (int)(it % W);
        const float2 d = *reinterpret_cast<const float2 *>(dseq + (size_t)it * 64 + 2 * cl);
        const size_t base = ((size_t)b * H * W + wc) * 64 + 2 * cl;
#pragma unroll 4
        for (int h = 0; h < H; ++h) {
            const size_t o = base + (size_t)h * W * 64;
            const float2 v = Act<T>::cvt2(Act<T>::ldraw2(y + o));
            const float z0 = fmaf(v.x, sc.x, sf.x), z1 = fmaf(v.y, sc.y, sf.y);
            const float2 gv = Act<T>::round2(make_float2(z0 > 0.f ? d.x * inv : 0.f, z1 > 0.f ? d.y * inv : 0.f));
            Act<T>::st2(g + o, gv);
            s1a += gv.x; s1b += gv.y;
            s2a = fmaf(gv.x, (v.x - mu.x) * rs.x, s2a);
            s2b = fmaf(gv.y, (v.y - mu.y) * rs.y, s2b);
        }
    }
    sh[grp * 128 + 2 * cl] = s1a;       sh[grp * 128 + 2 * cl + 1] = s1b;
    sh[grp * 128 + 64 + 2 * cl] = s2a;  sh[grp * 128 + 64 + 2 * cl + 1] = s2b;
    __syncthreads();
    if (threadIdx.x < 128) {
        float t = 0.f;
#pragma unroll
        for (int q = 0; q < 8; ++q) t += sh[q * 128 + threadIdx.x];
        stat_partials[(size_t)blockIdx.x * 128 + threadIdx.x] = t;
    }
}

}

extern "C" size_t ww_cnn_small_workspace_bytes(int B, int F, int T, int act_dtype) {
    if (B < 1 || F < 1 || T < 1) return 0;
    return make_layout(B, F, T, act_dtype).total;
}

extern "C" int ww_cnn_small_fwd(ww_ctx *ctx, int act_dtype, void *const *params, const float *x, int B, int F, int T, int training,
                                float bn_momentum, float bn_eps, float dropout_p, uint64_t seed, uint64_t step,
                                uint64_t sample_offset, void *ws, size_t ws_bytes, float *logits, ww_stream_t stream) {
    int rc = check_common("ww_cnn_small_fwd", ctx, act_dtype, params, x, B, F, T, ws, ws_bytes);
    if (rc) return rc;
    WW_REQUIRE(logits != nullptr, WW_E_INVALID, "ww_cnn_small_fwd: logits is null");
    const Layout L = make_layout(B, F, T, act_dtype);
    char *w = (char *)ws;
    auto Fp = [&](size_t off) { return (float *)(w + off); };
    rc = conv_stack_fwd(ctx, act_dtype, params, x, B, F, T, training, bn_momentum, bn_eps, L, w, stream);
    if (rc) return rc;
    rc = ww_gap_fwd(ctx, act_dtype, w + L.y[8], Fp(L.ss[8]), Fp(L.mr[8]), B, L.Ho, L.Wo, Fp(L.pool), stream);
    if (rc) return rc;
    return ww_head_fwd(ctx, Fp(L.pool), B, L.Ho * L.Wo, (const float *)params[45], (const float *)params[46], dropout_p,
                       training, seed, step, sample_offset, Fp(L.pd), logits, stream);
}

extern "C" int ww_cnn_small_bwd(ww_ctx *ctx, int act_dtype, void *const *params, void *const *grads, const float *x,
                                const float *dlogits, int B, int F, int T, float dropout_p, uint64_t seed, uint64_t step,
                                uint64_t sample_offset, void *ws, size_t ws_bytes, int part, ww_stream_t stream) {
    int rc = check_common("ww_cnn_small_bwd", ctx, act_dtype, params, x, B, F, T, ws, ws_bytes);
    if (rc) return rc;
    WW_REQUIRE(grads && dlogits, WW_E_INVALID, "ww_cnn_small_bwd: null argument");
    WW_REQUIRE(part == WW_BWD_ALL || part == WW_BWD_LATE || part == WW_BWD_EARLY, WW_E_INVALID,
               "ww_cnn_small_bwd: unknown part %d", part);
    const Layout L = make_layout(B, F, T, act_dtype);
    char *w = (char *)ws;
    auto Fp = [&](size_t off) { return (float *)(w + off); };
    auto G = [&](int i) { return (float *)grads[i]; };
    for (int l = 0; l < NL; ++l) {
        WW_REQUIRE(grads[widx(l)] && grads[bnidx(l)] && grads[bnidx(l) + 1], WW_E_INVALID,
                   "ww_cnn_small_bwd: missing gradient buffer for conv layer %d", l);
    }
    WW_REQUIRE(grads[45] && grads[46], WW_E_INVALID, "ww_cnn_small_bwd: missing classifier gradient buffers");
    const int HW = L.Ho * L.Wo;
    if (part != WW_BWD_EARLY) {
        rc = ww_head_bwd(ctx, dlogits, Fp(L.pd), Fp(L.pool), B, HW, (const float *)params[45], dropout_p, 1, seed, step,
                         sample_offset, (const float *)params[bnidx(8)], Fp(L.mr[8]), G(45), G(46), Fp(L.dpool),
                         Fp(L.coef[8]), G(bnidx(8)), G(bnidx(8) + 1), stream);
        if (rc) return rc;
    }
    return conv_stack_bwd(ctx, act_dtype, params, grads, x, B, F, T, L, w, true, stream, part);
}

extern "C" int ww_cnn_front_fwd(ww_ctx *ctx, int act_dtype, void *const *params, const float *x, int B, int F, int T, int training,
                                float bn_momentum, float bn_eps, void *ws, size_t ws_bytes, float *seq, ww_stream_t stream) {
    int rc = check_common("ww_cnn_front_fwd", ctx, act_dtype, params, x, B, F, T, ws, ws_bytes, 45);
    if (rc) return rc;
    WW_REQUIRE(seq != nullptr, WW_E_INVALID, "ww_cnn_front_fwd: seq is null");
    const Layout L = make_layout(B, F, T, act_dtype);
    char *w = (char *)ws;
    rc = conv_stack_fwd(ctx, act_dtype, params, x, B, F, T, training, bn_momentum, bn_eps, L, w, stream);
    if (rc) return rc;
    const long items = (long)B * L.Wo;
    const int grid = (int)std::min<long>((items + 7) / 8, 2048);
    hipStream_t st = (hipStream_t)stream;
    if (act_dtype == WW_ACT_BF16)
        hipLaunchKernelGGL(k_freqpool_fwd<ww_bf16>, dim3(grid), dim3(256), 0, st, (const ww_bf16 *)(w + L.y[8]),
                           (const float *)(w + L.ss[8]), B, L.Ho, L.Wo, seq);
    else if (act_dtype == WW_ACT_F16)
        hipLaunchKernelGGL(k_freqpool_fwd<ww_f16>, dim3(grid), dim3(256), 0, st, (const ww_f16 *)(w + L.y[8]),
                           (const float *)(w + L.ss[8]), B, L.Ho, L.Wo, seq);
    else
        hipLaunchKernelGGL(k_freqpool_fwd<float>, dim3(grid), dim3(256), 0, st, (const float *)(w + L.y[8]),
                           (const float *)(w + L.ss[8]), B, L.Ho, L.Wo, seq);
    WW_LAUNCH_CHECK();
    return WW_OK;
}

extern "C" int ww_cnn_front_bwd(ww_ctx *ctx, int act_dtype, void *const *params, void *const *grads, const float *x,
                                const float *dseq, int B, int F, int T, void *ws, size_t ws_bytes, ww_stream_t stream) {
    int rc = check_common("ww_cnn_front_bwd", ctx, act_dtype, params, x, B, F, T, ws, ws_bytes, 45);
    if (rc) return rc;
    WW_REQUIRE(grads && dseq, WW_E_INVALID, "ww_cnn_front_bwd: null argument");
    for (int l = 0; l < NL; ++l)
        WW_REQUIRE(grads[widx(l)] && grads[bnidx(l)] && grads[bnidx(l) + 1], WW_E_INVALID,
                   "ww_cnn_front_bwd: missing gradient buffer for conv layer %d", l);
    const Layout L = make_layout(B, F, T, act_dtype);
    char *w = (char *)ws;
    hipStream_t st = (hipStream_t)stream;
    float *stat = (float *)(w + L.scratch);
    const long items = (long)B * L.Wo;
    const int grid = (int)std::min<long>((items + 7) / 8, (long)WW_MAX_PARTIALS);
    if (act_dtype == WW_ACT_BF16)
        hipLaunchKernelGGL(k_freqpool_bwd<ww_bf16>, dim3(grid), dim3(256), 0, st, dseq, (const ww_bf16 *)(w + L.y[8]),
                           (const float *)(w + L.ss[8]), (const float *)(w + L.mr[8]), B, L.Ho, L.Wo, (ww_bf16 *)(w + L.g[0]), stat);
    else if (act_dtype == WW_ACT_F16)
        hipLaunchKernelGGL(k_freqpool_bwd<ww_f16>, dim3(grid), dim3(256), 0, st, dseq, (const ww_f16 *)(w + L.y[8]),
                           (const float *)(w + L.ss[8]), (const float *)(w + L.mr[8]), B, L.Ho, L.Wo, (ww_f16 *)(w + L.g[0]), stat);
    else
        hipLaunchKernelGGL(k_freqpool_bwd<float>, dim3(grid), dim3(256), 0, st, dseq, (const float *)(w + L.y[8]),
                           (const float *)(w + L.ss[8]), (const float *)(w + L.mr[8]), B, L.Ho, L.Wo, (float *)(w + L.g[0]), stat);
    WW_LAUNCH_CHECK();
    rc = ww_launch_bn_bwd_finalize(stat, grid, (double)B * L.Ho * L.Wo, (const float *)params[bnidx(8)],
                                   (const float *)(w + L.mr[8]), (float *)(w + L.coef[8]), (float *)grads[bnidx(8)],
                                   (float *)grads[bnidx(8) + 1], st);
    if (rc) return rc;
    return conv_stack_bwd(ctx, act_dtype, params, grads, x, B, F, T, L, w, false, stream);
}
```

Baseline: 421,600 samples/s.

## Fuse BatchNorm stat finalize into producer tail and consumer prologue

Each conv forward kernel now reduces its per-block BN partials in-kernel. A ticket counter per group lets the last block of each group fold the members into double-precision group sums. The separate BN finalize kernel launch is removed in training: the next layer's kernel (dw, pw, gap, freqpool) recomputes scale/shift from the group sums in its prologue, and block 0 writes the running stats. This removes one small launch and its serialization per BN layer, at the cost of atomics, extra per-block prologue work and new persistent ticket and group buffers.

Result: no change. 423,600 samples/s, median of 6 (+0.5%).

```diff
diff --git a/wakeword_trainer_home_amd/csrc/ww_bn_finish.h b/wakeword_trainer_home_amd/csrc/ww_bn_finish.h
--- /dev/null
+++ b/wakeword_trainer_home_amd/csrc/ww_bn_finish.h
@@ -0,0 +1,113 @@
+#pragma once
+#include "ww_internal.h"
+
+struct ww_bn_chain {
+    const double *grp;
+    int ng;
+    double count;
+    ww_bn_t bn;
+    float *ss, *mr;
+};
+
+struct ww_bn_fwd_consts { float scale, shift, mean, rstd, run_mean, run_var; };
+
+__host__ __device__ inline ww_bn_fwd_consts ww_bn_fwd_finish(double s, double q, double count, float gamma, float beta, float eps,
+                                                             float momentum, float run_mean, float run_var) {
+#pragma clang fp contract(off)
+    ww_bn_fwd_consts o;
+    const double mean = s / count;
+    double var = fma(-mean, mean, q / count);
+    if (var < 0.0) var = 0.0;
+    const double rstd = 1.0 / sqrt(var + (double)eps);
+    const double scale = (double)gamma * rstd;
+    o.scale = (float)scale;
+    o.shift = (float)fma(-mean, scale, (double)beta);
+    o.mean = (float)mean;
+    o.rstd = (float)rstd;
+    const double m = momentum;
+    const double unb = count > 1.0 ? var * count / (count - 1.0) : var;
+    o.run_mean = (float)fma(1.0 - m, (double)run_mean, m * mean);
+    o.run_var = (float)fma(1.0 - m, (double)run_var, m * unb);
+    return o;
+}
+
+int ww_conv_stem_fwd_impl(ww_ctx *ctx, int act_dtype, const float *x, const float *w, int B, int Hin, int Win, void *y,
+                          const ww_bn_t *bn, float *ss_out, float *mr_out, void *scratch, double *grp, ww_bn_chain *chain_out,
+                          ww_stream_t stream);
+int ww_dwconv3x3_fwd_impl(ww_ctx *ctx, int act_dtype, const void *y_in, const float *ss_in, const ww_bn_chain *chain_in,
+                          const float *w, int B, int H, int W, void *y, const ww_bn_t *bn, float *ss_out, float *mr_out,
+                          void *scratch, double *grp, ww_bn_chain *chain_out, ww_stream_t stream);
+int ww_pwconv1x1_fwd_impl(ww_ctx *ctx, int act_dtype, const void *y_in, const float *ss_in, const ww_bn_chain *chain_in,
+                          const float *w, int B, int H, int W, void *y, const ww_bn_t *bn, float *ss_out, float *mr_out,
+                          void *scratch, double *grp, ww_bn_chain *chain_out, ww_stream_t stream);
+int ww_gap_fwd_impl(ww_ctx *ctx, int act_dtype, const void *y, const float *ss, const float *mr, const ww_bn_chain *chain_in,
+                    int B, int H, int W, float *pool, ww_stream_t stream);
+
+#ifdef __HIPCC__
+static_assert(WW_MAX_PARTIALS <= 64 * WW_BN_NG_MAX, "ww_stat_tail: a group has at most 64 members (32 loads per thread)");
+
+__device__ __forceinline__ int ww_bn_groups(int grid) { return grid < WW_BN_NG_MAX ? grid : WW_BN_NG_MAX; }
+
+__device__ __forceinline__ void ww_stat_tail(float t, float *slab, double *grp, unsigned *cnt, float *sh) {
+    const int tid = threadIdx.x;
+    const int grid = (int)gridDim.x, ng = ww_bn_groups(grid), g = (int)blockIdx.x % ng;
+    const int members = (grid - g + ng - 1) / ng;
+    if (tid < 128) __hip_atomic_store(slab + (size_t)blockIdx.x * 128 + tid, t, __ATOMIC_RELAXED, __HIP_MEMORY_SCOPE_AGENT);
+    asm volatile("s_waitcnt vmcnt(0)" ::: "memory");
+    __syncthreads();
+    int *flag = reinterpret_cast<int *>(sh + 512);
+    if (tid == 0) {
+        unsigned *c = cnt + g * WW_TICKET_STRIDE;
+        const unsigned old = __hip_atomic_fetch_add(c, 1u, __ATOMIC_RELAXED, __HIP_MEMORY_SCOPE_AGENT);
+        const int last = old + 1u == (unsigned)members;
+        if (last) __hip_atomic_store(c, 0u, __ATOMIC_RELAXED, __HIP_MEMORY_SCOPE_AGENT);
+        *flag = last;
+    }
+    __syncthreads();
+    if (!*flag) return;
+    __builtin_amdgcn_fence(__ATOMIC_ACQUIRE, "wavefront");
+    const int col = tid & 127, par = tid >> 7;
+    float v[32];
+#pragma unroll
+    for (int j = 0; j < 32; ++j) {
+        const int m = min(par + 2 * j, members - 1);
+        v[j] = __hip_atomic_load(slab + (size_t)(g + m * ng) * 128 + col, __ATOMIC_RELAXED, __HIP_MEMORY_SCOPE_AGENT);
+    }
+    double a = 0.0;
+#pragma unroll
+    for (int j = 0; j < 32; ++j)
+        if (par + 2 * j < members) a += (double)v[j];
+    double *shd = reinterpret_cast<double *>(sh);
+    shd[tid] = a;
+    __syncthreads();
+    if (tid < 128) grp[(size_t)g * 128 + tid] = shd[tid] + shd[tid + 128];
+}
+
+__device__ __forceinline__ void ww_bn_prologue(const ww_bn_chain &ch, float *tab) {
+    const int c = threadIdx.x;
+    if (c < 64) {
+        const float gamma = ch.bn.gamma[c], beta = ch.bn.beta[c];
+        const bool upd = blockIdx.x == 0 && ch.bn.running_mean != nullptr;
+        const float rm = upd ? ch.bn.running_mean[c] : 0.f, rv = upd ? ch.bn.running_var[c] : 1.f;
+        double sv[WW_BN_NG_MAX], qv[WW_BN_NG_MAX];
+#pragma unroll
+        for (int g = 0; g < WW_BN_NG_MAX; ++g) {
+            const int gg = min(g, ch.ng - 1);
+            sv[g] = ch.grp[gg * 128 + c];
+            qv[g] = ch.grp[gg * 128 + 64 + c];
+        }
+        double s = 0.0, q = 0.0;
+#pragma unroll
+        for (int g = 0; g < WW_BN_NG_MAX; ++g)
+            if (g < ch.ng) { s += sv[g]; q += qv[g]; }
+        const ww_bn_fwd_consts k = ww_bn_fwd_finish(s, q, ch.count, gamma, beta, ch.bn.eps, ch.bn.momentum, rm, rv);
+        tab[c] = k.scale; tab[64 + c] = k.shift; tab[128 + c] = k.mean; tab[192 + c] = k.rstd;
+        if (blockIdx.x == 0) {
+            ch.ss[c] = k.scale; ch.ss[64 + c] = k.shift;
+            ch.mr[c] = k.mean; ch.mr[64 + c] = k.rstd;
+            if (upd) { ch.bn.running_mean[c] = k.run_mean; ch.bn.running_var[c] = k.run_var; }
+        }
+    }
+    __syncthreads();
+}
+#endif
diff --git a/wakeword_trainer_home_amd/csrc/ww_conv_fwd.hip b/wakeword_trainer_home_amd/csrc/ww_conv_fwd.hip
--- a/wakeword_trainer_home_amd/csrc/ww_conv_fwd.hip
+++ b/wakeword_trainer_home_amd/csrc/ww_conv_fwd.hip
@@ -1,5 +1,6 @@
 #include "ww_internal.h"
 #include "ww_act.h"
+#include "ww_bn_finish.h"
 
 namespace {
 
@@ -11,7 +12,7 @@
 }
 
 __device__ __forceinline__ void reduce_stats_slots(float s0, float s1, float q0, float q1, float *sh ,
-                                                   float *__restrict__ partial_row) {
+                                                   float *slab, double *grp, unsigned *cnt) {
     const int tid = threadIdx.x, slot = tid >> 5, cl = tid & 31;
     __syncthreads();
     sh[slot * 128 + 2 * cl] = s0;
@@ -19,19 +20,19 @@
     sh[slot * 128 + 64 + 2 * cl] = q0;
     sh[slot * 128 + 64 + 2 * cl + 1] = q1;
     __syncthreads();
+    float t = 0.f;
     if (tid < 128) {
-        float t = 0.f;
 #pragma unroll
         for (int s = 0; s < 8; ++s) t += sh[s * 128 + tid];
-        partial_row[tid] = t;
-    }
+    }
+    ww_stat_tail(t, slab, grp, cnt, sh);
 }
 
 template <typename T>
 __global__ __launch_bounds__(256) void k_stem_fwd(const float *__restrict__ x, const float *__restrict__ w, int B,
                                                   int Hin, int Win, int Ho, int Wo, T *__restrict__ y,
-                                                  float *__restrict__ partials, int rev) {
-    __shared__ float sh[32 * 128];
+                                                  float *partials, double *grp, unsigned *cnt, int rev) {
+    __shared__ __align__(16) float sh[32 * 128];
     extern __shared__ float xs[];
     const int tid = threadIdx.x, px = tid >> 3, c8 = tid & 7;
     const int ld = Win + 2;
@@ -108,12 +109,12 @@
             sh[px * 128 + 64 + 8 * c8 + j] = q[j];
         }
         __syncthreads();
+        float t = 0.f;
         if (tid < 128) {
-            float t = 0.f;
 #pragma unroll 8
             for (int i = 0; i < 32; ++i) t += sh[i * 128 + tid];
-            partials[(size_t)blockIdx.x * 128 + tid] = t;
-        }
+        }
+        ww_stat_tail(t, partials, grp, cnt, sh);
     }
 }
 
@@ -177,8 +178,8 @@
 template <typename T>
 __global__ __launch_bounds__(256) void k_dw_fwd(const T *__restrict__ yin, const float *__restrict__ ss,
                                                 const float *__restrict__ w, DwGeom g, T *__restrict__ y,
-                                                float *__restrict__ partials) {
-    __shared__ float sh[8 * 128];
+                                                float *partials, double *grp, unsigned *cnt, ww_bn_chain ch) {
+    __shared__ __align__(16) float sh[8 * 128];
     typedef typename Act<T>::raw2 raw2;
     const int tid = threadIdx.x, slot = tid >> 5, cl = tid & 31;
     float wa[9], wb[9];
@@ -187,8 +188,10 @@
         wa[t] = w[(2 * cl) * 9 + t];
         wb[t] = w[(2 * cl + 1) * 9 + t];
     }
-    const float2 sc = *reinterpret_cast<const float2 *>(ss + 2 * cl);
-    const float2 sf = *reinterpret_cast<const float2 *>(ss + 64 + 2 * cl);
+    const float *ssp = ss;
+    if (ch.grp) { ww_bn_prologue(ch, sh); ssp = sh; }
+    const float2 sc = *reinterpret_cast<const float2 *>(ssp + 2 * cl);
+    const float2 sf = *reinterpret_cast<const float2 *>(ssp + 64 + 2 * cl);
     float s0 = 0.f, s1 = 0.f, q0 = 0.f, q1 = 0.f;
     const size_t img_stride = (size_t)g.H * g.W * 64;
     for (long item = (long)blockIdx.x * 8 + slot; item < g.items; item += (long)gridDim.x * 8) {
@@ -223,7 +226,7 @@
           }
         }
     }
-    if (partials) reduce_stats_slots(s0, s1, q0, q1, sh, partials + (size_t)blockIdx.x * 128);
+    if (partials) reduce_stats_slots(s0, s1, q0, q1, sh, partials, grp, cnt);
 }
 
 constexpr int PW_TILE = 128;
@@ -232,7 +235,7 @@
 template <typename T>
 __global__ __launch_bounds__(256) void k_pw_fwd(const T *__restrict__ yin, const float *__restrict__ ss,
                                                 const float *__restrict__ w, long M, T *__restrict__ y,
-                                                float *__restrict__ partials) {
+                                                float *partials, double *grp, unsigned *cnt, ww_bn_chain ch) {
     extern __shared__ __align__(16) float pw_lds[];
     float *tile = pw_lds;
     float *otile = pw_lds + PW_TILE * PW_LD;
@@ -247,8 +250,6 @@
         wreg[4 * s4] = v.x; wreg[4 * s4 + 1] = v.y; wreg[4 * s4 + 2] = v.z; wreg[4 * s4 + 3] = v.w;
     }
     const int c4 = tid & 15;
-    const float4 sc = *reinterpret_cast<const float4 *>(ss + 4 * c4);
-    const float4 sf = *reinterpret_cast<const float4 *>(ss + 64 + 4 * c4);
     float s1 = 0.f, s2 = 0.f;
     const long ntiles = (M + PW_TILE - 1) / PW_TILE;
     raw4 raw[8];
@@ -261,6 +262,11 @@
         }
     };
     if ((long)blockIdx.x < ntiles) issue(blockIdx.x);
+    const float *ssp = ss;
+    if (ch.grp) { ww_bn_prologue(ch, tile); ssp = tile; }
+    const float4 sc = *reinterpret_cast<const float4 *>(ssp + 4 * c4);
+    const float4 sf = *reinterpret_cast<const float4 *>(ssp + 64 + 4 * c4);
+    if (ch.grp) __syncthreads();
     for (long ti = blockIdx.x; ti < ntiles; ti += gridDim.x) {
         const long p0 = ti * PW_TILE;
 #pragma unroll
@@ -321,10 +327,12 @@
             sh[wv * 64 + 32 + r] = s2;
         }
         __syncthreads();
+        float t = 0.f;
         if (tid < 128) {
             const int kind = tid >> 6, c = tid & 63, nn = c >> 5, rr = c & 31;
-            partials[(size_t)blockIdx.x * 128 + tid] = sh[nn * 64 + kind * 32 + rr] + sh[(2 + nn) * 64 + kind * 32 + rr];
-        }
+            t = sh[nn * 64 + kind * 32 + rr] + sh[(2 + nn) * 64 + kind * 32 + rr];
+        }
+        ww_stat_tail(t, partials, grp, cnt, sh);
     }
 }
 
@@ -333,7 +341,7 @@
 template <typename H>
 __global__ __launch_bounds__(256) void k_pw_fwd_bf16(const H *__restrict__ yin, const float *__restrict__ ss,
                                                      const float *__restrict__ w, long M, H *__restrict__ y,
-                                                     float *__restrict__ partials, int rev) {
+                                                     float *partials, double *grp, unsigned *cnt, ww_bn_chain ch, int rev) {
     extern __shared__ __align__(16) unsigned char pwh_lds[];
     H *atile = reinterpret_cast<H *>(pwh_lds);
     H *otile = atile + PW_TILE * PWH_LD;
@@ -351,8 +359,6 @@
         wb[t] = ww_pack8<H>(v);
     }
     const int c4 = tid & 15;
-    const float4 sc = *reinterpret_cast<const float4 *>(ss + 4 * c4);
-    const float4 sf = *reinterpret_cast<const float4 *>(ss + 64 + 4 * c4);
     float s1 = 0.f, s2 = 0.f;
     const long ntiles = (M + PW_TILE - 1) / PW_TILE;
     typename A16::raw4 raw[8];
@@ -366,6 +372,11 @@
         }
     };
     if ((long)blockIdx.x < ntiles) issue(blockIdx.x);
+    const float *ssp = ss;
+    if (ch.grp) { ww_bn_prologue(ch, reinterpret_cast<float *>(pwh_lds)); ssp = reinterpret_cast<const float *>(pwh_lds); }
+    const float4 sc = *reinterpret_cast<const float4 *>(ssp + 4 * c4);
+    const float4 sf = *reinterpret_cast<const float4 *>(ssp + 64 + 4 * c4);
+    if (ch.grp) __syncthreads();
     for (long ti = blockIdx.x; ti < ntiles; ti += gridDim.x) {
         const long p0 = (rev ? ntiles - 1 - ti : ti) * PW_TILE;
 #pragma unroll
@@ -416,22 +427,28 @@
             sh[wv * 64 + 32 + r] = s2;
         }
         __syncthreads();
+        float t = 0.f;
         if (tid < 128) {
             const int kind = tid >> 6, c = tid & 63, nn = c >> 5, rr = c & 31;
-            partials[(size_t)blockIdx.x * 128 + tid] = sh[nn * 64 + kind * 32 + rr] + sh[(2 + nn) * 64 + kind * 32 + rr];
-        }
+            t = sh[nn * 64 + kind * 32 + rr] + sh[(2 + nn) * 64 + kind * 32 + rr];
+        }
+        ww_stat_tail(t, partials, grp, cnt, sh);
     }
 }
 
 template <typename T>
 __global__ __launch_bounds__(1024) void k_gap_fwd(const T *__restrict__ y, const float *__restrict__ ss,
-                                                  const float *__restrict__ mr, int HW, float *__restrict__ pool) {
+                                                  const float *__restrict__ mr, int HW, float *__restrict__ pool,
+                                                  ww_bn_chain ch) {
     __shared__ __align__(16) float sh[64 * 192];
     const int tid = threadIdx.x, slot = tid >> 4, cl = tid & 15, b = blockIdx.x;
-    const float4 sc = *reinterpret_cast<const float4 *>(ss + 4 * cl);
-    const float4 sf = *reinterpret_cast<const float4 *>(ss + 64 + 4 * cl);
-    const float4 mu = *reinterpret_cast<const float4 *>(mr + 4 * cl);
-    const float4 rs = *reinterpret_cast<const float4 *>(mr + 64 + 4 * cl);
+    const float *ssp = ss, *mrp = mr;
+    if (ch.grp) { ww_bn_prologue(ch, sh); ssp = sh; mrp = sh + 128; }
+    const float4 sc = *reinterpret_cast<const float4 *>(ssp + 4 * cl);
+    const float4 sf = *reinterpret_cast<const float4 *>(ssp + 64 + 4 * cl);
+    const float4 mu = *reinterpret_cast<const float4 *>(mrp + 4 * cl);
+    const float4 rs = *reinterpret_cast<const float4 *>(mrp + 64 + 4 * cl);
+    if (ch.grp) __syncthreads();
     const T *yb = y + (size_t)b * HW * 64 + 4 * cl;
     float4 a = make_float4(0.f, 0.f, 0.f, 0.f), h = a, c = a;
     auto one = [](float v, float scv, float sfv, float muv, float rsv, float &av, float &hv, float &cv) {
@@ -495,12 +512,21 @@
     }
 }
 
-int finish_bn(ww_ctx *ctx, const float *partials, int rows, double count, const ww_bn_t *bn, float *ss_out,
-              float *mr_out, hipStream_t st) {
+int finish_bn(ww_ctx *ctx, double *grp, int rows, double count, const ww_bn_t *bn, float *ss_out, float *mr_out,
+              ww_bn_chain *chain, hipStream_t st) {
+    if (chain) *chain = ww_bn_chain{nullptr, 0, count, *bn, ss_out, mr_out};
+    const int ng = rows < WW_BN_NG_MAX ? rows : WW_BN_NG_MAX;
+    if (bn->training && chain) {
+        chain->grp = grp;
+        chain->ng = ng;
+        return WW_OK;
+    }
     ww_prof_scope ps_(ctx, WW_K_FINALIZE, st);
-    if (bn->training) return ww_launch_bn_fwd_finalize(partials, rows, count, bn, ss_out, mr_out, st);
+    if (bn->training) return ww_launch_bn_fwd_finish(grp, ng, count, bn, ss_out, mr_out, st);
     return ww_launch_bn_eval_ss(bn, ss_out, mr_out, st);
 }
+
+const ww_bn_chain kNoChain = {nullptr, 0, 0.0, ww_bn_t{}, nullptr, nullptr};
 
 int check_bn(const char *who, const ww_bn_t *bn, const float *ss_out, const float *mr_out, const void *scratch) {
     WW_REQUIRE(bn && bn->gamma && bn->beta && ss_out && mr_out, WW_E_INVALID, "%s: null BatchNorm argument", who);
@@ -517,7 +543,7 @@
 
 template <typename T>
 int launch_stem_fwd(ww_ctx *ctx, const float *x, const float *w, int B, int Hin, int Win, void *y, float *partials,
-                    int *grid_out, hipStream_t st) {
+                    double *grp, int *grid_out, hipStream_t st) {
     const int Ho = (Hin + 1) / 2, Wo = (Win + 1) / 2;
     const long nrows = (long)B * ((Ho + 1) / 2);
     const size_t smem = (size_t)5 * (Win + 2) * sizeof(float);
@@ -525,7 +551,8 @@
     {
         ww_prof_scope ps_(ctx, WW_K_STEM_FWD, st);
         static const int rev = ww_env_int("WW_STEM_FWD_REV", 1);
-        hipLaunchKernelGGL(k_stem_fwd<T>, dim3(grid), dim3(256), smem, st, x, w, B, Hin, Win, Ho, Wo, (T *)y, partials, rev);
+        hipLaunchKernelGGL(k_stem_fwd<T>, dim3(grid), dim3(256), smem, st, x, w, B, Hin, Win, Ho, Wo, (T *)y, partials, grp,
+                           ww_tickets(ctx, WW_SITE_STEM_FWD), rev);
     }
     WW_LAUNCH_CHECK();
     *grid_out = grid;
@@ -533,13 +560,14 @@
 }
 
 template <typename T>
-int launch_dw_fwd(ww_ctx *ctx, const void *y_in, const float *ss_in, const float *w, const DwGeom &g, void *y,
-                  float *partials, int *grid_out, hipStream_t st) {
+int launch_dw_fwd(ww_ctx *ctx, const void *y_in, const float *ss_in, const ww_bn_chain &ch, const float *w, const DwGeom &g,
+                  void *y, float *partials, double *grp, int *grid_out, hipStream_t st) {
     const long nblk = (g.items + 7) / 8;
     const int grid = ww_occupancy_grid((const void *)k_dw_fwd<T>, 256, 0, nblk, WW_MAX_PARTIALS);
     {
         ww_prof_scope ps_(ctx, WW_K_DW_FWD, st);
-        hipLaunchKernelGGL(k_dw_fwd<T>, dim3(grid), dim3(256), 0, st, (const T *)y_in, ss_in, w, g, (T *)y, partials);
+        hipLaunchKernelGGL(k_dw_fwd<T>, dim3(grid), dim3(256), 0, st, (const T *)y_in, ss_in, w, g, (T *)y, partials, grp,
+                           ww_tickets(ctx, WW_SITE_DW_FWD), ch);
     }
     WW_LAUNCH_CHECK();
     *grid_out = grid;
@@ -547,15 +575,16 @@
 }
 
 template <typename H>
-int launch_pw_fwd_bf16(ww_ctx *ctx, const void *y_in, const float *ss_in, const float *w, long M, void *y,
-                       float *partials, int *grid_out, hipStream_t st) {
+int launch_pw_fwd_bf16(ww_ctx *ctx, const void *y_in, const float *ss_in, const ww_bn_chain &ch, const float *w, long M, void *y,
+                       float *partials, double *grp, int *grid_out, hipStream_t st) {
     const long ntiles = (M + PW_TILE - 1) / PW_TILE;
     const size_t smem = (size_t)2 * PW_TILE * PWH_LD * 2;
     const int grid = ww_occupancy_grid((const void *)k_pw_fwd_bf16<H>, 256, smem, ntiles, WW_MAX_PARTIALS);
     {
         ww_prof_scope ps_(ctx, WW_K_PW_FWD, st);
         static const int rev = ww_env_int("WW_PW_FWD_REV", 1);
-        hipLaunchKernelGGL(k_pw_fwd_bf16<H>, dim3(grid), dim3(256), smem, st, (const H *)y_in, ss_in, w, M, (H *)y, partials, rev);
+        hipLaunchKernelGGL(k_pw_fwd_bf16<H>, dim3(grid), dim3(256), smem, st, (const H *)y_in, ss_in, w, M, (H *)y, partials,
+                           grp, ww_tickets(ctx, WW_SITE_PW_FWD), ch, rev);
     }
     WW_LAUNCH_CHECK();
     *grid_out = grid;
@@ -563,15 +592,16 @@
 }
 
 template <typename T>
-int launch_pw_fwd(ww_ctx *ctx, const void *y_in, const float *ss_in, const float *w, long M, void *y, float *partials,
-                  int *grid_out, hipStream_t st) {
+int launch_pw_fwd(ww_ctx *ctx, const void *y_in, const float *ss_in, const ww_bn_chain &ch, const float *w, long M, void *y,
+                  float *partials, double *grp, int *grid_out, hipStream_t st) {
     const long ntiles = (M + PW_TILE - 1) / PW_TILE;
     const size_t smem = (size_t)(Act<T>::is_f32 ? 1 : 2) * PW_TILE * PW_LD * sizeof(float);
     WW_HIP(hipFuncSetAttribute((const void *)k_pw_fwd<T>, hipFuncAttributeMaxDynamicSharedMemorySize, (int)smem));
     const int grid = ww_occupancy_grid((const void *)k_pw_fwd<T>, 256, smem, ntiles, WW_MAX_PARTIALS);
     {
         ww_prof_scope ps_(ctx, WW_K_PW_FWD, st);
-        hipLaunchKernelGGL(k_pw_fwd<T>, dim3(grid), dim3(256), smem, st, (const T *)y_in, ss_in, w, M, (T *)y, partials);
+        hipLaunchKernelGGL(k_pw_fwd<T>, dim3(grid), dim3(256), smem, st, (const T *)y_in, ss_in, w, M, (T *)y, partials, grp,
+                           ww_tickets(ctx, WW_SITE_PW_FWD), ch);
     }
     WW_LAUNCH_CHECK();
     *grid_out = grid;
@@ -580,9 +610,9 @@
 
 }
 
-extern "C" int ww_conv_stem_fwd(ww_ctx *ctx, int act_dtype, const float *x, const float *w, int B, int Hin, int Win,
-                                void *y, const ww_bn_t *bn, float *ss_out, float *mr_out, void *scratch,
-                                ww_stream_t stream) {
+int ww_conv_stem_fwd_impl(ww_ctx *ctx, int act_dtype, const float *x, const float *w, int B, int Hin, int Win, void *y,
+                          const ww_bn_t *bn, float *ss_out, float *mr_out, void *scratch, double *grp, ww_bn_chain *chain_out,
+                          ww_stream_t stream) {
     WW_REQUIRE(ctx && x && w && y, WW_E_INVALID, "ww_conv_stem_fwd: null argument");
     WW_REQUIRE(B >= 1 && Hin >= 1 && Win >= 1, WW_E_INVALID, "ww_conv_stem_fwd: bad shape (%d,%d,%d)", B, Hin, Win);
     int rc = check_bn("ww_conv_stem_fwd", bn, ss_out, mr_out, scratch);
@@ -590,16 +620,23 @@
     hipStream_t st = (hipStream_t)stream;
     float *partials = bn->training ? (float *)scratch : nullptr;
     int grid = 0;
-    rc = act_dtype == WW_ACT_BF16  ? launch_stem_fwd<ww_bf16>(ctx, x, w, B, Hin, Win, y, partials, &grid, st)
-         : act_dtype == WW_ACT_F16 ? launch_stem_fwd<ww_f16>(ctx, x, w, B, Hin, Win, y, partials, &grid, st)
-                                   : launch_stem_fwd<float>(ctx, x, w, B, Hin, Win, y, partials, &grid, st);
+    if (!grp && partials) grp = ww_scratch_grp(scratch);
+    rc = act_dtype == WW_ACT_BF16  ? launch_stem_fwd<ww_bf16>(ctx, x, w, B, Hin, Win, y, partials, grp, &grid, st)
+         : act_dtype == WW_ACT_F16 ? launch_stem_fwd<ww_f16>(ctx, x, w, B, Hin, Win, y, partials, grp, &grid, st)
+                                   : launch_stem_fwd<float>(ctx, x, w, B, Hin, Win, y, partials, grp, &grid, st);
     if (rc) return rc;
-    return finish_bn(ctx, partials, grid, (double)B * ((Hin + 1) / 2) * ((Win + 1) / 2), bn, ss_out, mr_out, st);
-}
-
-extern "C" int ww_dwconv3x3_fwd(ww_ctx *ctx, int act_dtype, const void *y_in, const float *ss_in, const float *w,
-                                int B, int H, int W, void *y, const ww_bn_t *bn, float *ss_out, float *mr_out,
-                                void *scratch, ww_stream_t stream) {
+    return finish_bn(ctx, grp, grid, (double)B * ((Hin + 1) / 2) * ((Win + 1) / 2), bn, ss_out, mr_out, chain_out, st);
+}
+extern "C" int ww_conv_stem_fwd(ww_ctx *ctx, int act_dtype, const float *x, const float *w, int B, int Hin, int Win,
+                                void *y, const ww_bn_t *bn, float *ss_out, float *mr_out, void *scratch,
+                                ww_stream_t stream) {
+    return ww_conv_stem_fwd_impl(ctx, act_dtype, x, w, B, Hin, Win, y, bn, ss_out, mr_out, scratch, nullptr, nullptr, stream);
+}
+
+int ww_dwconv3x3_fwd_impl(ww_ctx *ctx, int act_dtype, const void *y_in, const float *ss_in, const ww_bn_chain *chain_in,
+                          const float *w, int B, int H, int W, void *y, const ww_bn_t *bn, float *ss_out, float *mr_out,
+                          void *scratch, double *grp, ww_bn_chain *chain_out, ww_stream_t stream) {
+    const ww_bn_chain &ch = chain_in ? *chain_in : kNoChain;
     WW_REQUIRE(ctx && y_in && ss_in && w && y, WW_E_INVALID, "ww_dwconv3x3_fwd: null argument");
     WW_REQUIRE(B >= 1 && H >= 1 && W >= 1, WW_E_INVALID, "ww_dwconv3x3_fwd: bad shape (%d,%d,%d)", B, H, W);
     WW_REQUIRE((long)H * W * 64 < (1L << 31), WW_E_UNSUPPORTED, "ww_dwconv3x3_fwd: one image of %d x %d x 64 exceeds 2^31 elements", H, W);
@@ -614,16 +651,24 @@
     hipStream_t st = (hipStream_t)stream;
     float *partials = bn->training ? (float *)scratch : nullptr;
     int grid = 0;
-    rc = act_dtype == WW_ACT_BF16  ? launch_dw_fwd<ww_bf16>(ctx, y_in, ss_in, w, g, y, partials, &grid, st)
-         : act_dtype == WW_ACT_F16 ? launch_dw_fwd<ww_f16>(ctx, y_in, ss_in, w, g, y, partials, &grid, st)
-                                   : launch_dw_fwd<float>(ctx, y_in, ss_in, w, g, y, partials, &grid, st);
+    if (!grp && partials) grp = ww_scratch_grp(scratch);
+    rc = act_dtype == WW_ACT_BF16  ? launch_dw_fwd<ww_bf16>(ctx, y_in, ss_in, ch, w, g, y, partials, grp, &grid, st)
+         : act_dtype == WW_ACT_F16 ? launch_dw_fwd<ww_f16>(ctx, y_in, ss_in, ch, w, g, y, partials, grp, &grid, st)
+                                   : launch_dw_fwd<float>(ctx, y_in, ss_in, ch, w, g, y, partials, grp, &grid, st);
     if (rc) return rc;
-    return finish_bn(ctx, partials, grid, (double)B * H * W, bn, ss_out, mr_out, st);
-}
-
-extern "C" int ww_pwconv1x1_fwd(ww_ctx *ctx, int act_dtype, const void *y_in, const float *ss_in, const float *w,
+    return finish_bn(ctx, grp, grid, (double)B * H * W, bn, ss_out, mr_out, chain_out, st);
+}
+extern "C" int ww_dwconv3x3_fwd(ww_ctx *ctx, int act_dtype, const void *y_in, const float *ss_in, const float *w,
                                 int B, int H, int W, void *y, const ww_bn_t *bn, float *ss_out, float *mr_out,
                                 void *scratch, ww_stream_t stream) {
+    return ww_dwconv3x3_fwd_impl(ctx, act_dtype, y_in, ss_in, nullptr, w, B, H, W, y, bn, ss_out, mr_out, scratch, nullptr,
+                                 nullptr, stream);
+}
+
+int ww_pwconv1x1_fwd_impl(ww_ctx *ctx, int act_dtype, const void *y_in, const float *ss_in, const ww_bn_chain *chain_in,
+                          const float *w, int B, int H, int W, void *y, const ww_bn_t *bn, float *ss_out, float *mr_out,
+                          void *scratch, double *grp, ww_bn_chain *chain_out, ww_stream_t stream) {
+    const ww_bn_chain &ch = chain_in ? *chain_in : kNoChain;
     WW_REQUIRE(ctx && y_in && ss_in && w && y, WW_E_INVALID, "ww_pwconv1x1_fwd: null argument");
     WW_REQUIRE(B >= 1 && H >= 1 && W >= 1, WW_E_INVALID, "ww_pwconv1x1_fwd: bad shape (%d,%d,%d)", B, H, W);
     int rc = check_bn("ww_pwconv1x1_fwd", bn, ss_out, mr_out, scratch);
@@ -632,15 +677,23 @@
     hipStream_t st = (hipStream_t)stream;
     float *partials = bn->training ? (float *)scratch : nullptr;
     int grid = 0;
-    rc = act_dtype == WW_ACT_BF16  ? launch_pw_fwd_bf16<ww_bf16>(ctx, y_in, ss_in, w, M, y, partials, &grid, st)
-         : act_dtype == WW_ACT_F16 ? launch_pw_fwd_bf16<ww_f16>(ctx, y_in, ss_in, w, M, y, partials, &grid, st)
-                                   : launch_pw_fwd<float>(ctx, y_in, ss_in, w, M, y, partials, &grid, st);
+    if (!grp && partials) grp = ww_scratch_grp(scratch);
+    rc = act_dtype == WW_ACT_BF16  ? launch_pw_fwd_bf16<ww_bf16>(ctx, y_in, ss_in, ch, w, M, y, partials, grp, &grid, st)
+         : act_dtype == WW_ACT_F16 ? launch_pw_fwd_bf16<ww_f16>(ctx, y_in, ss_in, ch, w, M, y, partials, grp, &grid, st)
+                                   : launch_pw_fwd<float>(ctx, y_in, ss_in, ch, w, M, y, partials, grp, &grid, st);
     if (rc) return rc;
-    return finish_bn(ctx, partials, grid, (double)M, bn, ss_out, mr_out, st);
-}
-
-extern "C" int ww_gap_fwd(ww_ctx *ctx, int act_dtype, const void *y, const float *ss, const float *mr, int B, int H,
-                          int W, float *pool, ww_stream_t stream) {
+    return finish_bn(ctx, grp, grid, (double)M, bn, ss_out, mr_out, chain_out, st);
+}
+extern "C" int ww_pwconv1x1_fwd(ww_ctx *ctx, int act_dtype, const void *y_in, const float *ss_in, const float *w,
+                                int B, int H, int W, void *y, const ww_bn_t *bn, float *ss_out, float *mr_out,
+                                void *scratch, ww_stream_t stream) {
+    return ww_pwconv1x1_fwd_impl(ctx, act_dtype, y_in, ss_in, nullptr, w, B, H, W, y, bn, ss_out, mr_out, scratch, nullptr,
+                                 nullptr, stream);
+}
+
+int ww_gap_fwd_impl(ww_ctx *ctx, int act_dtype, const void *y, const float *ss, const float *mr, const ww_bn_chain *chain_in,
+                    int B, int H, int W, float *pool, ww_stream_t stream) {
+    const ww_bn_chain &ch = chain_in ? *chain_in : kNoChain;
     WW_REQUIRE(ctx && y && ss && mr && pool, WW_E_INVALID, "ww_gap_fwd: null argument");
     WW_REQUIRE(B >= 1 && H >= 1 && W >= 1, WW_E_INVALID, "ww_gap_fwd: bad shape (%d,%d,%d)", B, H, W);
     int rc = check_act("ww_gap_fwd", act_dtype);
@@ -649,14 +702,18 @@
     {
         ww_prof_scope ps_(ctx, WW_K_GAP_FWD, st);
         if (act_dtype == WW_ACT_BF16)
-            hipLaunchKernelGGL(k_gap_fwd<ww_bf16>, dim3(B), dim3(1024), 0, st, (const ww_bf16 *)y, ss, mr, H * W, pool);
+            hipLaunchKernelGGL(k_gap_fwd<ww_bf16>, dim3(B), dim3(1024), 0, st, (const ww_bf16 *)y, ss, mr, H * W, pool, ch);
         else if (act_dtype == WW_ACT_F16)
-            hipLaunchKernelGGL(k_gap_fwd<ww_f16>, dim3(B), dim3(1024), 0, st, (const ww_f16 *)y, ss, mr, H * W, pool);
+            hipLaunchKernelGGL(k_gap_fwd<ww_f16>, dim3(B), dim3(1024), 0, st, (const ww_f16 *)y, ss, mr, H * W, pool, ch);
         else
-            hipLaunchKernelGGL(k_gap_fwd<float>, dim3(B), dim3(1024), 0, st, (const float *)y, ss, mr, H * W, pool);
+            hipLaunchKernelGGL(k_gap_fwd<float>, dim3(B), dim3(1024), 0, st, (const float *)y, ss, mr, H * W, pool, ch);
     }
     WW_LAUNCH_CHECK();
     return WW_OK;
+}
+extern "C" int ww_gap_fwd(ww_ctx *ctx, int act_dtype, const void *y, const float *ss, const float *mr, int B, int H,
+                          int W, float *pool, ww_stream_t stream) {
+    return ww_gap_fwd_impl(ctx, act_dtype, y, ss, mr, nullptr, B, H, W, pool, stream);
 }
 
 extern "C" int ww_head_fwd(ww_ctx *ctx, const float *pool, int B, int HW, const float *fc_w, const float *fc_b,
diff --git a/wakeword_trainer_home_amd/csrc/ww_ctx.hip b/wakeword_trainer_home_amd/csrc/ww_ctx.hip
--- a/wakeword_trainer_home_amd/csrc/ww_ctx.hip
+++ b/wakeword_trainer_home_amd/csrc/ww_ctx.hip
@@ -5,6 +5,7 @@
 #include <vector>
 
 #include "ww_internal.h"
+#include "ww_bn_finish.h"
 #include <algorithm>
 
 static thread_local char g_err[512] = "";
@@ -52,6 +53,23 @@
     c->logmel_wgs = 0;
     c->tw16k = nullptr;
     c->norm_partials = nullptr;
+    c->tickets = nullptr;
+    {
+        int cur = 0;
+        const size_t bytes = (size_t)WW_SITE_N * WW_BN_NG_MAX * WW_TICKET_STRIDE * sizeof(unsigned);
+        hipError_t e = hipGetDevice(&cur);
+        if (e == hipSuccess) e = hipSetDevice(device);
+        if (e == hipSuccess) e = hipMalloc((void **)&c->tickets, bytes);
+        if (e == hipSuccess) e = hipMemset(c->tickets, 0, bytes);
+        if (e == hipSuccess) e = hipDeviceSynchronize();
+        (void)hipSetDevice(cur);
+        if (e != hipSuccess) {
+            ww_set_error("ww_ctx_create: ticket counters: %s", hipGetErrorString(e));
+            if (c->tickets) (void)hipFree(c->tickets);
+            delete c;
+            return WW_E_HIP;
+        }
+    }
     c->defer_on = 0;
     c->deferred = new std::vector<ww_reduce_item>();
     c->prof_recs = new std::vector<ww_prof_rec>();
@@ -109,6 +127,7 @@
     free_tables(ctx->tables);
     if (ctx->tw16k) (void)hipFree(ctx->tw16k);
     if (ctx->norm_partials) (void)hipFree(ctx->norm_partials);
+    if (ctx->tickets) (void)hipFree(ctx->tickets);
     for (auto *v : {ctx->prof_recs, ctx->prof_free}) {
         for (auto &r : *v) { (void)hipEventDestroy(r.a); (void)hipEventDestroy(r.b); }
         delete v;
@@ -404,7 +423,7 @@
 }
 
 extern "C" size_t ww_layer_scratch_bytes(void) {
-    return (size_t)(WW_STAT_SLAB_FLOATS + WW_DW_SLAB_FLOATS) * sizeof(float);
+    return (size_t)(WW_STAT_SLAB_FLOATS + WW_DW_SLAB_FLOATS + WW_GRP_FLOATS) * sizeof(float);
 }
 
 
@@ -443,36 +462,9 @@
     __syncthreads();
 }
 
-__global__ __launch_bounds__(1024) void k_bn_fwd_finalize(const float *__restrict__ partials, int rows,
-                                                          double count, ww_bn_t bn, float *__restrict__ ss,
-                                                          float *__restrict__ mr) {
-    __shared__ double sh[256][16];
-    __shared__ double tot[16];
-    float g_c = 0.f, b_c = 0.f, rm_c = 0.f, rv_c = 1.f;
-    if (threadIdx.x < 8) {
-        const int c = 8 * blockIdx.x + threadIdx.x;
-        g_c = bn.gamma[c]; b_c = bn.beta[c];
-        if (bn.running_mean) { rm_c = bn.running_mean[c]; rv_c = bn.running_var[c]; }
-    }
-    ww_colgroup_sum(partials, rows, blockIdx.x, sh, tot);
-    if (threadIdx.x < 8) {
-        const int c = 8 * blockIdx.x + threadIdx.x;
-        const double mean = tot[threadIdx.x] / count;
-        double var = tot[8 + threadIdx.x] / count - mean * mean;
-        if (var < 0.0) var = 0.0;
-        const double rstd = 1.0 / sqrt(var + (double)bn.eps);
-        const double scale = (double)g_c * rstd;
-        ss[c] = (float)scale;
-        ss[64 + c] = (float)((double)b_c - mean * scale);
-        mr[c] = (float)mean;
-        mr[64 + c] = (float)rstd;
-        if (bn.running_mean) {
-            const double m = bn.momentum;
-            const double unb = count > 1.0 ? var * count / (count - 1.0) : var;
-            bn.running_mean[c] = (float)((1.0 - m) * (double)rm_c + m * mean);
-            bn.running_var[c] = (float)((1.0 - m) * (double)rv_c + m * unb);
-        }
-    }
+__global__ __launch_bounds__(64) void k_bn_fwd_finish(ww_bn_chain ch) {
+    __shared__ float tab[256];
+    ww_bn_prologue(ch, tab);
 }
 
 __global__ void k_bn_eval_ss(ww_bn_t bn, float *__restrict__ ss, float *__restrict__ mr) {
@@ -563,9 +555,10 @@
     }
 }
 
-int ww_launch_bn_fwd_finalize(const float *partials, int rows, double count, const ww_bn_t *bn, float *ss_out,
-                              float *mr_out, hipStream_t st) {
-    hipLaunchKernelGGL(k_bn_fwd_finalize, dim3(8), dim3(1024), 0, st, partials, rows, count, *bn, ss_out, mr_out);
+int ww_launch_bn_fwd_finish(const double *grp, int ng, double count, const ww_bn_t *bn, float *ss_out, float *mr_out,
+                            hipStream_t st) {
+    ww_bn_chain ch{grp, ng, count, *bn, ss_out, mr_out};
+    hipLaunchKernelGGL(k_bn_fwd_finish, dim3(1), dim3(64), 0, st, ch);
     WW_LAUNCH_CHECK();
     return WW_OK;
 }
diff --git a/wakeword_trainer_home_amd/csrc/ww_internal.h b/wakeword_trainer_home_amd/csrc/ww_internal.h
--- a/wakeword_trainer_home_amd/csrc/ww_internal.h
+++ b/wakeword_trainer_home_amd/csrc/ww_internal.h
@@ -74,6 +74,7 @@
     ww_feat_tables *tables;
     float2 *tw16k;
     double *norm_partials;
+    unsigned *tickets;
     const ww_step_ctl *step_ctl;
     int logmel_wgs;
     uint32_t prof_mask;
@@ -110,9 +111,17 @@
 #define WW_STAT_SLAB_FLOATS (WW_MAX_PARTIALS * 128)
 #define WW_DW_SLAB_ROWS 768
 #define WW_DW_SLAB_FLOATS (WW_DW_SLAB_ROWS * 4096)
+#define WW_BN_NG_MAX 16
+#define WW_GRP_FLOATS (WW_BN_NG_MAX * 128 * 2)
+#define WW_TICKET_STRIDE 32
+enum { WW_SITE_STEM_FWD = 0, WW_SITE_DW_FWD, WW_SITE_PW_FWD, WW_SITE_N };
+static inline unsigned *ww_tickets(ww_ctx *ctx, int site) { return ctx->tickets + (size_t)site * WW_BN_NG_MAX * WW_TICKET_STRIDE; }
+static inline double *ww_scratch_grp(void *scratch) {
+    return reinterpret_cast<double *>(static_cast<float *>(scratch) + WW_STAT_SLAB_FLOATS + WW_DW_SLAB_FLOATS);
+}
 
-int ww_launch_bn_fwd_finalize(const float *partials, int rows, double count, const ww_bn_t *bn, float *ss_out,
-                              float *mr_out, hipStream_t st);
+int ww_launch_bn_fwd_finish(const double *grp, int ng, double count, const ww_bn_t *bn, float *ss_out, float *mr_out,
+                            hipStream_t st);
 int ww_launch_bn_eval_ss(const ww_bn_t *bn, float *ss_out, float *mr_out, hipStream_t st);
 int ww_launch_bn_bwd_finalize(const float *partials, int rows, double count, const float *gamma,
                               const float *mr, float *coef_out, float *dgamma, float *dbeta, hipStream_t st);
diff --git a/wakeword_trainer_home_amd/csrc/ww_model.hip b/wakeword_trainer_home_amd/csrc/ww_model.hip
--- a/wakeword_trainer_home_amd/csrc/ww_model.hip
+++ b/wakeword_trainer_home_amd/csrc/ww_model.hip
@@ -1,5 +1,6 @@
 #include "ww_internal.h"
 #include "ww_act.h"
+#include "ww_bn_finish.h"
 #include <algorithm>
 
 namespace {
@@ -9,7 +10,7 @@
 struct Layout {
     int Ho, Wo;
     size_t A;
-    size_t y[NL], g[2], ss[NL], mr[NL], coef[NL], pool, pd, dpool, scratch, total;
+    size_t y[NL], g[2], ss[NL], mr[NL], coef[NL], grp[NL], pool, pd, dpool, scratch, total;
 };
 
 Layout make_layout(int B, int F, int T, int act_dtype) {
@@ -28,7 +29,8 @@
     L.pool = take((size_t)B * 192);
     L.pd = take((size_t)B * 64);
     L.dpool = take((size_t)B * 64);
-    L.scratch = take(WW_STAT_SLAB_FLOATS + WW_DW_SLAB_FLOATS);
+    L.scratch = take(WW_STAT_SLAB_FLOATS + WW_DW_SLAB_FLOATS + WW_GRP_FLOATS);
+    for (int i = 0; i < NL; ++i) L.grp[i] = take(WW_GRP_FLOATS);
     L.total = o;
     return L;
 }
@@ -64,24 +66,29 @@
 }
 
 int conv_stack_fwd(ww_ctx *ctx, int act_dtype, void *const *params, const float *x, int B, int F, int T, int training,
-                   float bn_momentum, float bn_eps, const Layout &L, char *w, ww_stream_t stream) {
-    auto Fp = [&](size_t off) { return (float *)(w + off); };
+                   float bn_momentum, float bn_eps, const Layout &L, char *w, ww_bn_chain *last, ww_stream_t stream) {
+    auto Fp = [&](size_t off) { return (float *)(w + off); };
+    auto Gp = [&](int l) { return (double *)(w + L.grp[l]); };
     void *scratch = w + L.scratch;
+    ww_bn_chain ch, nx;
     ww_bn_t bn = make_bn(params, 0, training, bn_momentum, bn_eps);
-    int rc = ww_conv_stem_fwd(ctx, act_dtype, x, (const float *)params[0], B, F, T, w + L.y[0], &bn, Fp(L.ss[0]), Fp(L.mr[0]),
-                              scratch, stream);
+    int rc = ww_conv_stem_fwd_impl(ctx, act_dtype, x, (const float *)params[0], B, F, T, w + L.y[0], &bn, Fp(L.ss[0]),
+                                   Fp(L.mr[0]), scratch, Gp(0), &ch, stream);
     if (rc) return rc;
     for (int i = 0; i < 4; ++i) {
         const int ld = 1 + 2 * i, lp = 2 + 2 * i;
         bn = make_bn(params, ld, training, bn_momentum, bn_eps);
-        rc = ww_dwconv3x3_fwd(ctx, act_dtype, w + L.y[ld - 1], Fp(L.ss[ld - 1]), (const float *)params[widx(ld)], B, L.Ho,
-                              L.Wo, w + L.y[ld], &bn, Fp(L.ss[ld]), Fp(L.mr[ld]), scratch, stream);
-        if (rc) return rc;
+        rc = ww_dwconv3x3_fwd_impl(ctx, act_dtype, w + L.y[ld - 1], Fp(L.ss[ld - 1]), &ch, (const float *)params[widx(ld)], B,
+                                   L.Ho, L.Wo, w + L.y[ld], &bn, Fp(L.ss[ld]), Fp(L.mr[ld]), scratch, Gp(ld), &nx, stream);
+        if (rc) return rc;
+        ch = nx;
         bn = make_bn(params, lp, training, bn_momentum, bn_eps);
-        rc = ww_pwconv1x1_fwd(ctx, act_dtype, w + L.y[ld], Fp(L.ss[ld]), (const float *)params[widx(lp)], B, L.Ho, L.Wo,
-                              w + L.y[lp], &bn, Fp(L.ss[lp]), Fp(L.mr[lp]), scratch, stream);
-        if (rc) return rc;
-    }
+        rc = ww_pwconv1x1_fwd_impl(ctx, act_dtype, w + L.y[ld], Fp(L.ss[ld]), &ch, (const float *)params[widx(lp)], B, L.Ho,
+                                   L.Wo, w + L.y[lp], &bn, Fp(L.ss[lp]), Fp(L.mr[lp]), scratch, Gp(lp), &nx, stream);
+        if (rc) return rc;
+        ch = nx;
+    }
+    *last = ch;
     return WW_OK;
 }
 
@@ -119,10 +126,13 @@
 
 template <typename T>
 __global__ __launch_bounds__(256) void k_freqpool_fwd(const T *__restrict__ y, const float *__restrict__ ss, int B, int H, int W,
-                                                      float *__restrict__ seq) {
+                                                      float *__restrict__ seq, ww_bn_chain ch) {
+    __shared__ float tab[256];
     const int grp = threadIdx.x >> 5, cl = threadIdx.x & 31;
-    const float2 sc = *reinterpret_cast<const float2 *>(ss + 2 * cl);
-    const float2 sf = *reinterpret_cast<const float2 *>(ss + 64 + 2 * cl);
+    const float *ssp = ss;
+    if (ch.grp) { ww_bn_prologue(ch, tab); ssp = tab; }
+    const float2 sc = *reinterpret_cast<const float2 *>(ssp + 2 * cl);
+    const float2 sf = *reinterpret_cast<const float2 *>(ssp + 64 + 2 * cl);
     const float inv = 1.0f / (float)H;
     for (long it = (long)blockIdx.x * 8 + grp; it < (long)B * W; it += (long)gridDim.x * 8) {
         const long b = it / W;
@@ -195,9 +205,10 @@
     const Layout L = make_layout(B, F, T, act_dtype);
     char *w = (char *)ws;
     auto Fp = [&](size_t off) { return (float *)(w + off); };
-    rc = conv_stack_fwd(ctx, act_dtype, params, x, B, F, T, training, bn_momentum, bn_eps, L, w, stream);
-    if (rc) return rc;
-    rc = ww_gap_fwd(ctx, act_dtype, w + L.y[8], Fp(L.ss[8]), Fp(L.mr[8]), B, L.Ho, L.Wo, Fp(L.pool), stream);
+    ww_bn_chain last;
+    rc = conv_stack_fwd(ctx, act_dtype, params, x, B, F, T, training, bn_momentum, bn_eps, L, w, &last, stream);
+    if (rc) return rc;
+    rc = ww_gap_fwd_impl(ctx, act_dtype, w + L.y[8], Fp(L.ss[8]), Fp(L.mr[8]), &last, B, L.Ho, L.Wo, Fp(L.pool), stream);
     if (rc) return rc;
     return ww_head_fwd(ctx, Fp(L.pool), B, L.Ho * L.Wo, (const float *)params[45], (const float *)params[46], dropout_p,
                        training, seed, step, sample_offset, Fp(L.pd), logits, stream);
@@ -237,20 +248,21 @@
     WW_REQUIRE(seq != nullptr, WW_E_INVALID, "ww_cnn_front_fwd: seq is null");
     const Layout L = make_layout(B, F, T, act_dtype);
     char *w = (char *)ws;
-    rc = conv_stack_fwd(ctx, act_dtype, params, x, B, F, T, training, bn_momentum, bn_eps, L, w, stream);
+    ww_bn_chain last;
+    rc = conv_stack_fwd(ctx, act_dtype, params, x, B, F, T, training, bn_momentum, bn_eps, L, w, &last, stream);
     if (rc) return rc;
     const long items = (long)B * L.Wo;
     const int grid = (int)std::min<long>((items + 7) / 8, 2048);
     hipStream_t st = (hipStream_t)stream;
     if (act_dtype == WW_ACT_BF16)
         hipLaunchKernelGGL(k_freqpool_fwd<ww_bf16>, dim3(grid), dim3(256), 0, st, (const ww_bf16 *)(w + L.y[8]),
-                           (const float *)(w + L.ss[8]), B, L.Ho, L.Wo, seq);
+                           (const float *)(w + L.ss[8]), B, L.Ho, L.Wo, seq, last);
     else if (act_dtype == WW_ACT_F16)
         hipLaunchKernelGGL(k_freqpool_fwd<ww_f16>, dim3(grid), dim3(256), 0, st, (const ww_f16 *)(w + L.y[8]),
-                           (const float *)(w + L.ss[8]), B, L.Ho, L.Wo, seq);
+                           (const float *)(w + L.ss[8]), B, L.Ho, L.Wo, seq, last);
     else
         hipLaunchKernelGGL(k_freqpool_fwd<float>, dim3(grid), dim3(256), 0, st, (const float *)(w + L.y[8]),
-                           (const float *)(w + L.ss[8]), B, L.Ho, L.Wo, seq);
+                           (const float *)(w + L.ss[8]), B, L.Ho, L.Wo, seq, last);
     WW_LAUNCH_CHECK();
     return WW_OK;
 }
```
